# yanyan-li/PlanarSLAM

Measured on NVIDIA H100. Metric: rgbd_frames_per_sec_640x480, higher is better.
Workload: dtype u8/f64

## Files before the change

planarslam_b200/csrc/peac_kernels.cuh:

```cuda
#pragma once
#include <cuda_runtime.h>

#include <cfloat>
#include <cstdint>

#include "pslam_internal.h"

namespace pslam {

#define PEAC_MAX_PLANES 128
#define PEAC_PL_WORDS (PEAC_MAX_PLANES / 32)

__device__ __forceinline__ void eig33sym_jacobi(const double K[3][3], double s[3], double V[3][3]) {
    double a[3][3], d[3], b[3], z[3];
#pragma unroll
    for (int i = 0; i < 3; ++i) {
#pragma unroll
        for (int j = 0; j < 3; ++j) { a[i][j] = K[i][j]; V[i][j] = (i == j) ? 1.0 : 0.0; }
        d[i] = b[i] = a[i][i];
        z[i] = 0.0;
    }
    for (int sweep = 0; sweep < 50; ++sweep) {
        const double sm = fabs(a[0][1]) + fabs(a[0][2]) + fabs(a[1][2]);
        if (sm == 0.0) break;
        const double tresh = (sweep < 3) ? 0.2 * sm / 9.0 : 0.0;
#pragma unroll
        for (int p = 0; p < 2; ++p)
#pragma unroll
            for (int q = p + 1; q < 3; ++q) {
                const double g = 100.0 * fabs(a[p][q]);
                if (sweep > 3 && fabs(d[p]) + g == fabs(d[p]) && fabs(d[q]) + g == fabs(d[q])) {
                    a[p][q] = 0.0;
                } else if (fabs(a[p][q]) > tresh) {
                    double h = d[q] - d[p], t;
                    if (fabs(h) + g == fabs(h)) {
                        t = a[p][q] / h;
                    } else {
                        const double theta = 0.5 * h / a[p][q];
                        t = 1.0 / (fabs(theta) + sqrt(1.0 + theta * theta));
                        if (theta < 0.0) t = -t;
                    }
                    const double c = 1.0 / sqrt(1.0 + t * t), sn = t * c, tau = sn / (1.0 + c);
                    h = t * a[p][q];
                    z[p] -= h; z[q] += h; d[p] -= h; d[q] += h;
                    a[p][q] = 0.0;
#define PEAC_ROT(i, j, k, l) { const double gg = a[i][j], hh = a[k][l]; a[i][j] = gg - sn * (hh + gg * tau); a[k][l] = hh + sn * (gg - hh * tau); }
                    if (p == 0 && q == 1) { PEAC_ROT(0, 2, 1, 2) }
                    else if (p == 0 && q == 2) { PEAC_ROT(0, 1, 1, 2) }
                    else { PEAC_ROT(0, 1, 0, 2) }
#undef PEAC_ROT
#pragma unroll
                    for (int j = 0; j < 3; ++j) {
                        const double gg = V[j][p], hh = V[j][q];
                        V[j][p] = gg - sn * (hh + gg * tau);
                        V[j][q] = hh + sn * (gg - hh * tau);
                    }
                }
            }
#pragma unroll
        for (int i = 0; i < 3; ++i) { b[i] += z[i]; d[i] = b[i]; z[i] = 0.0; }
    }
#define PEAC_CSWAP(i, j) if (d[j] < d[i]) { double t_ = d[i]; d[i] = d[j]; d[j] = t_; \
        t_ = V[0][i]; V[0][i] = V[0][j]; V[0][j] = t_; t_ = V[1][i]; V[1][i] = V[1][j]; V[1][j] = t_; t_ = V[2][i]; V[2][i] = V[2][j]; V[2][j] = t_; }
    PEAC_CSWAP(0, 1)
    PEAC_CSWAP(0, 2)
    PEAC_CSWAP(1, 2)
#undef PEAC_CSWAP
    s[0] = d[0]; s[1] = d[1]; s[2] = d[2];
}

__device__ __forceinline__ void peac_stats_compute(const double st[9], int N, double geo[8]) {
    const double sc = 1.0 / N;
    const double sx = st[0], sy = st[1], sz = st[2];
    geo[0] = sx * sc; geo[1] = sy * sc; geo[2] = sz * sc;
    double K[3][3];
    K[0][0] = st[3] - sx * sx * sc; K[0][1] = st[6] - sx * sy * sc; K[0][2] = st[8] - sx * sz * sc;
    K[1][1] = st[4] - sy * sy * sc; K[1][2] = st[7] - sy * sz * sc; K[2][2] = st[5] - sz * sz * sc;
    K[1][0] = K[0][1]; K[2][0] = K[0][2]; K[2][1] = K[1][2];
    double sv[3], V[3][3];
    eig33sym_jacobi(K, sv, V);
    if (V[0][0] * geo[0] + V[1][0] * geo[1] + V[2][0] * geo[2] <= 0) { geo[3] = V[0][0]; geo[4] = V[1][0]; geo[5] = V[2][0]; }
    else { geo[3] = -V[0][0]; geo[4] = -V[1][0]; geo[5] = -V[2][0]; }
    geo[6] = sv[0] * sc;
    geo[7] = sv[0] / (sv[0] + sv[1] + sv[2]);
}

__device__ __forceinline__ double peac_t_mse(const PeacGeom& g, double tol, double z) { const double v = g.depth_sigma * z * z + tol; return v * v; }
__device__ __forceinline__ double peac_t_ang_init(const PeacGeom& g, double z) {
    if (z <= g.z_near) return g.t_ang_init_near;
    const double cz = fmin(z, g.z_far);
    const double factor = (g.angle_far - g.angle_near) / (g.z_far - g.z_near);
    return cos(factor * cz + g.angle_near - factor * g.z_near);
}
__device__ __forceinline__ double peac_sim(const double* ga, const double* gb) {
    return fabs(ga[3] * gb[3] + ga[4] * gb[4] + ga[5] * gb[5]);
}

__global__ void __launch_bounds__(128) k_peac_blocks(PeacGeom g, const uint16_t* __restrict__ depth, double* __restrict__ blk_st,
                                                     double* __restrict__ blk_geo, int32_t* __restrict__ blk_n, uint8_t* __restrict__ blk_valid) {
    const int b = blockIdx.x * 128 + threadIdx.x, frame = blockIdx.y;
    if (b >= g.nblk) return;
    const int bi = b / g.nbw, bj = b - bi * g.nbw;
    const uint16_t* D = depth + (size_t)frame * g.w * g.h;
    const double scale = (double)g.scale, fx = (double)g.fx, fy = (double)g.fy, cx = (double)g.cx, cy = (double)g.cy;
    double st[9] = {0, 0, 0, 0, 0, 0, 0, 0, 0};
    int n = 0;
    bool valid = true;
    for (int i = bi * g.win, ic = 0; ic < g.win && i < g.h && valid; ++i, ++ic)
        for (int j = bj * g.win, jc = 0; jc < g.win && j < g.w; ++j, ++jc) {
            const int dv = D[(size_t)i * g.w + j];
            if (dv == 0) { valid = false; break; }
            const double z = (double)dv * scale;
            const double tdz = g.depth_alpha * fabs(z) + g.depth_change_tol;
            if (j + 1 < g.w) { const int dn = D[(size_t)i * g.w + j + 1]; if (dn != 0 && fabs(z - (double)dn * scale) > tdz) { valid = false; break; } }
            if (i + 1 < g.h) { const int dn = D[(size_t)(i + 1) * g.w + j]; if (dn != 0 && fabs(z - (double)dn * scale) > tdz) { valid = false; break; } }
            const double x = ((double)j - cx) * z / fx, y = ((double)i - cy) * z / fy;
            st[0] += x; st[1] += y; st[2] += z;
            st[3] += x * x; st[4] += y * y; st[5] += z * z;
            st[6] += x * y; st[7] += y * z; st[8] += x * z;
            ++n;
        }
    double geo[8] = {0, 0, 0, 0, 0, 0, 0, 0};
    bool keep = false;
    if (!valid) { n = 0; for (int k = 0; k < 9; ++k) st[k] = 0; }
    if (n >= 4) {
        peac_stats_compute(st, n, geo);
        keep = valid && geo[6] < peac_t_mse(g, g.std_tol_init, geo[2]);
    } else {
        geo[6] = geo[7] = __longlong_as_double(0x7ff8000000000000LL);
    }
    const size_t o = (size_t)frame * g.nblk + b;
    for (int k = 0; k < 9; ++k) blk_st[o * 9 + k] = st[k];
    for (int k = 0; k < 8; ++k) blk_geo[o * 8 + k] = geo[k];
    blk_n[o] = n;
    blk_valid[o] = keep ? 1 : 0;
}

struct AhcState {
    int nslots;
    int words;
    double* st;
    double* geo;
    int32_t* N;
    int32_t* rid;
    int32_t* cid;
    uint8_t* alive;
    uint32_t* adj;
    int16_t* wlo;
    int16_t* whi;
    uint16_t* heap;
    float* keyf;
    int32_t* nb_list;
    int32_t* ds_parent;
    int32_t* ds_size;
};

__device__ __forceinline__ int ds_find(int32_t* parent, int x) {
    int r = x;
    while (parent[r] != r) r = parent[r];
    while (parent[x] != r) { const int nx = parent[x]; parent[x] = r; x = nx; }
    return r;
}
__device__ __forceinline__ void ds_union(int32_t* parent, int32_t* size, int x, int y) {
    const int xr = ds_find(parent, x), yr = ds_find(parent, y);
    if (xr == yr) return;
    if (size[xr] < size[yr]) { parent[xr] = yr; size[yr] += size[xr]; }
    else { parent[yr] = xr; size[xr] += size[yr]; }
}

struct HeapKey {
    const float* kf; const double* geo;
    __device__ __forceinline__ bool comp(int a, int b) const {
        const float fa = kf[a], fb = kf[b];
        if (fb < fa) return true;
        if (fb > fa) return false;
        return geo[(size_t)b * 8 + 6] < geo[(size_t)a * 8 + 6];
    }
};
__device__ __forceinline__ void heap_sift_up(uint16_t* h, const HeapKey& key, int hole, int top, int value) {
    int parent = (hole - 1) / 2;
    while (hole > top && key.comp(h[parent], value)) { h[hole] = h[parent]; hole = parent; parent = (hole - 1) / 2; }
    h[hole] = (uint16_t)value;
}
__device__ __forceinline__ void heap_push(uint16_t* h, int& len, const HeapKey& key, int id) { h[len] = (uint16_t)id; ++len; heap_sift_up(h, key, len - 1, 0, id); }
__device__ __forceinline__ int heap_pop(uint16_t* h, int& len, const HeapKey& key) {
    const int top = h[0], value = h[len - 1];
    --len;
    if (len > 0) {
        int hole = 0, child = 0;
        while (child < (len - 1) / 2) {
            child = 2 * (child + 1);
            if (key.comp(h[child], h[child - 1])) --child;
            h[hole] = h[child]; hole = child;
        }
        if ((len & 1) == 0 && child == (len - 2) / 2) { child = 2 * (child + 1); h[hole] = h[child - 1]; hole = child - 1; }
        heap_sift_up(h, key, hole, 0, value);
    }
    return top;
}

__device__ void ahc_run(const PeacGeom& g, AhcState S, int heap_len, int& next_cid, uint16_t* ex, const int exs, int& n_ex, bool& overflow) {
    const int lane = threadIdx.x & 31;
    const uint32_t full = 0xffffffffu;
    const HeapKey hkey{S.keyf, S.geo};
    int step = 0;
    while (heap_len > 0 && step <= g.max_step) {
        int p = 0;
        if (lane == 0) p = heap_pop(S.heap, heap_len, hkey);
        p = __shfl_sync(full, p, 0);
        heap_len = __shfl_sync(full, heap_len, 0);
        if (!S.alive[p]) continue;
        const int plo = S.wlo[p], phi = S.whi[p];
        int cnt = 0;
        for (int w0 = plo; w0 <= phi; w0 += 32) {
            const int w = w0 + lane;
            uint32_t bits = (w <= phi) ? S.adj[(size_t)p * S.words + w] : 0u;
            const int c = __popc(bits);
            int inc = c;
#pragma unroll
            for (int o = 1; o < 32; o <<= 1) { const int t = __shfl_up_sync(full, inc, o); if (lane >= o) inc += t; }
            int pos = cnt + inc - c;
            while (bits) { const int bpos = __ffs(bits) - 1; bits &= bits - 1; S.nb_list[pos++] = w * 32 + bpos; }
            cnt += __shfl_sync(full, inc, 31);
        }
        __syncwarp();
        const double* gp = S.geo + (size_t)p * 8;
        const double* sp = S.st + (size_t)p * 9;
        const int Np = S.N[p];
        double bst[9], bgeo[8];
        int best_nb = -1, best_cid = 0x7fffffff, best_N = 0;
#pragma unroll
        for (int k = 0; k < 8; ++k) bgeo[k] = 0;
        for (int i = lane; i < cnt; i += 32) {
            const int q = S.nb_list[i];
            const double* gq = S.geo + (size_t)q * 8;
            if (peac_sim(gp, gq) < g.sim_merge) continue;
            double st[9], geo[8];
            const double* sq = S.st + (size_t)q * 9;
#pragma unroll
            for (int k = 0; k < 9; ++k) st[k] = sp[k] + sq[k];
            const int Nq = S.N[q];
            peac_stats_compute(st, Np + Nq, geo);
            const int cq = S.cid[q];
            if (best_nb < 0 || geo[6] < bgeo[6] || (geo[6] == bgeo[6] && cq < best_cid)) {
                best_nb = q; best_cid = cq; best_N = Np + Nq;
#pragma unroll
                for (int k = 0; k < 9; ++k) bst[k] = st[k];
#pragma unroll
                for (int k = 0; k < 8; ++k) bgeo[k] = geo[k];
            }
        }
        double w_mse = bgeo[6];
        int w_nb = best_nb, w_cid = best_cid;
#pragma unroll
        for (int o = 16; o; o >>= 1) {
            const double om = __shfl_xor_sync(full, w_mse, o);
            const int onb = __shfl_xor_sync(full, w_nb, o), oc = __shfl_xor_sync(full, w_cid, o);
            if (onb >= 0 && (w_nb < 0 || om < w_mse || (om == w_mse && oc < w_cid))) { w_mse = om; w_nb = onb; w_cid = oc; }
        }
        bool merged = false;
        if (w_nb >= 0) {
            const int nb = w_nb;
            const int src = __ffs(__ballot_sync(full, best_nb == nb)) - 1;
            double st[9], geo[8];
#pragma unroll
            for (int k = 0; k < 9; ++k) st[k] = __shfl_sync(full, bst[k], src);
#pragma unroll
            for (int k = 0; k < 8; ++k) geo[k] = __shfl_sync(full, bgeo[k], src);
            const int Nc = __shfl_sync(full, best_N, src);
            if (geo[6] < peac_t_mse(g, g.std_tol_merge, geo[2])) {
                merged = true;
                const int rid_c = Np >= S.N[nb] ? S.rid[p] : S.rid[nb];
                if (lane == 0) ds_union(S.ds_parent, S.ds_size, S.rid[p], S.rid[nb]);
                const int nlo = S.wlo[nb], nhi = S.whi[nb];
                for (int w = nlo + lane; w <= nhi; w += 32) {
                    uint32_t bits = S.adj[(size_t)nb * S.words + w];
                    while (bits) {
                        const int q = w * 32 + __ffs(bits) - 1;
                        bits &= bits - 1;
                        if (q == p) continue;
                        atomicAnd(&S.adj[(size_t)q * S.words + (nb >> 5)], ~(1u << (nb & 31)));
                        atomicOr(&S.adj[(size_t)q * S.words + (p >> 5)], 1u << (p & 31));
                        if ((p >> 5) < S.wlo[q]) S.wlo[q] = (int16_t)(p >> 5);
                        if ((p >> 5) > S.whi[q]) S.whi[q] = (int16_t)(p >> 5);
                    }
                }
                __syncwarp();
                const int clo = min(plo, nlo), chi = max(phi, nhi);
                for (int w = clo + lane; w <= chi; w += 32) {
                    uint32_t u = S.adj[(size_t)p * S.words + w] | S.adj[(size_t)nb * S.words + w];
                    if (w == (p >> 5)) u &= ~(1u << (p & 31));
                    if (w == (nb >> 5)) u &= ~(1u << (nb & 31));
                    S.adj[(size_t)p * S.words + w] = u;
                    S.adj[(size_t)nb * S.words + w] = 0u;
                }
                if (lane == 0) {
#pragma unroll
                    for (int k = 0; k < 9; ++k) S.st[(size_t)p * 9 + k] = st[k];
#pragma unroll
                    for (int k = 0; k < 8; ++k) S.geo[(size_t)p * 8 + k] = geo[k];
                    S.N[p] = Nc; S.rid[p] = rid_c; S.cid[p] = next_cid; S.alive[nb] = 0; S.keyf[p] = (float)geo[6];
                    S.wlo[p] = (int16_t)clo; S.whi[p] = (int16_t)chi;
                }
                ++next_cid;
                __syncwarp();
                if (lane == 0) heap_push(S.heap, heap_len, hkey, p);
                heap_len = __shfl_sync(full, heap_len, 0);
            }
        }
        if (!merged) {
            if (Np >= g.min_support) { if (n_ex < PEAC_MAX_PLANES) { if (lane == 0) ex[n_ex * exs] = (uint16_t)p; ++n_ex; } else overflow = true; }
            for (int w = plo + lane; w <= phi; w += 32) {
                uint32_t bits = S.adj[(size_t)p * S.words + w];
                while (bits) { const int q = w * 32 + __ffs(bits) - 1; bits &= bits - 1; atomicAnd(&S.adj[(size_t)q * S.words + (p >> 5)], ~(1u << (p & 31))); }
                S.adj[(size_t)p * S.words + w] = 0u;
            }
            if (lane == 0) S.alive[p] = 0;
        }
        __syncwarp();
        ++step;
    }
    while (heap_len > 0) {
        int p = 0;
        if (lane == 0) p = heap_pop(S.heap, heap_len, hkey);
        p = __shfl_sync(full, p, 0);
        heap_len = __shfl_sync(full, heap_len, 0);
        if (S.alive[p] && S.N[p] >= g.min_support) { if (n_ex < PEAC_MAX_PLANES) { if (lane == 0) ex[n_ex * exs] = (uint16_t)p; ++n_ex; } else overflow = true; }
    }
    __syncwarp();
    if (lane == 0)
        for (int i = 1; i < n_ex; ++i) {
            const int v = ex[i * exs];
            int j = i - 1;
            while (j >= 0 && S.N[ex[j * exs]] < S.N[v]) { ex[(j + 1) * exs] = ex[j * exs]; --j; }
            ex[(j + 1) * exs] = (uint16_t)v;
        }
    __syncwarp();
}

struct PeacPlaneRec {
    double normal[3], center[3], mse, curvature;
    double st[9];
    int32_t N, rid, cid, valid;
};

template <int OCC>
__global__ void __launch_bounds__(32, OCC) k_peac_cluster(PeacGeom g, const double* __restrict__ blk_st, const double* __restrict__ blk_geo,
                                                     const int32_t* __restrict__ blk_n, const uint8_t* __restrict__ blk_valid,
                                                     double* node_st, double* node_geo, int32_t* node_n, int32_t* node_rid, int32_t* node_cid,
                                                     uint8_t* node_alive, uint32_t* adj, int16_t* wlo_all, int16_t* whi_all, int32_t* nb_list, int32_t* ds_parent,
                                                     int32_t* ds_size, PeacPlaneRec* planes, int32_t* n_planes, int32_t* blk_map,
                                                     int32_t* next_cid_out, int32_t* status, float* keyf_all) {
    const int frame = blockIdx.x, lane = threadIdx.x;
    const size_t fo = (size_t)frame * g.nblk;
    AhcState S;
    S.nslots = g.nblk; S.words = g.adj_words;
    S.st = node_st + fo * 9; S.geo = node_geo + fo * 8; S.N = node_n + fo; S.rid = node_rid + fo; S.cid = node_cid + fo;
    extern __shared__ __align__(16) unsigned char cluster_smem[];
    if (OCC > 12) {
        S.keyf = keyf_all + fo;
        S.heap = reinterpret_cast<uint16_t*>(cluster_smem);
    } else {
        S.keyf = reinterpret_cast<float*>(cluster_smem);
        S.heap = reinterpret_cast<uint16_t*>(cluster_smem + (size_t)g.nblk * sizeof(float));
    }
    S.alive = node_alive + fo; S.adj = adj + fo * g.adj_words; S.nb_list = nb_list + fo;
    S.wlo = wlo_all + fo; S.whi = whi_all + fo;
    S.ds_parent = ds_parent + fo; S.ds_size = ds_size + fo;
    const uint8_t* valid = blk_valid + fo;
    for (int b = lane; b < g.nblk; b += 32) {
        for (int k = 0; k < 9; ++k) S.st[(size_t)b * 9 + k] = blk_st[(fo + b) * 9 + k];
        for (int k = 0; k < 8; ++k) S.geo[(size_t)b * 8 + k] = blk_geo[(fo + b) * 8 + k];
        S.N[b] = blk_n[fo + b]; S.rid[b] = b; S.cid[b] = b; S.alive[b] = valid[b];
        S.ds_parent[b] = b; S.ds_size[b] = 1;
        S.keyf[b] = (float)blk_geo[(fo + b) * 8 + 6];
        S.wlo[b] = (int16_t)(max(b - g.nbw, 0) >> 5); S.whi[b] = (int16_t)(min(b + g.nbw, g.nblk - 1) >> 5);
    }
    __syncwarp();
    auto connect = [&](int a, int b) {
        atomicOr(&S.adj[(size_t)a * S.words + (b >> 5)], 1u << (b & 31));
        atomicOr(&S.adj[(size_t)b * S.words + (a >> 5)], 1u << (a & 31));
    };
    const int Nh = g.nbh, Nw = g.nbw;
    for (int i = lane; i < Nh; i += 32)
        for (int j = 1; j < Nw; j += 2) {
            const int c = i * Nw + j;
            if (!valid[c - 1]) { --j; continue; }
            if (!valid[c]) continue;
            if (j < Nw - 1 && !valid[c + 1]) { ++j; continue; }
            const double th = peac_t_ang_init(g, S.geo[(size_t)c * 8 + 2]);
            if ((j < Nw - 1 && peac_sim(S.geo + (size_t)(c - 1) * 8, S.geo + (size_t)(c + 1) * 8) >= th) ||
                (j == Nw - 1 && peac_sim(S.geo + (size_t)c * 8, S.geo + (size_t)(c - 1) * 8) >= th)) {
                connect(c, c - 1);
                if (j < Nw - 1) connect(c, c + 1);
            } else {
                --j;
            }
        }
    for (int j = lane; j < Nw; j += 32)
        for (int i = 1; i < Nh; i += 2) {
            const int c = i * Nw + j;
            if (!valid[c - Nw]) { --i; continue; }
            if (!valid[c]) continue;
            if (i < Nh - 1 && !valid[c + Nw]) { ++i; continue; }
            const double th = peac_t_ang_init(g, S.geo[(size_t)c * 8 + 2]);
            if ((i < Nh - 1 && peac_sim(S.geo + (size_t)(c - Nw) * 8, S.geo + (size_t)(c + Nw) * 8) >= th) ||
                (i == Nh - 1 && peac_sim(S.geo + (size_t)c * 8, S.geo + (size_t)(c - Nw) * 8) >= th)) {
                connect(c, c - Nw);
                if (i < Nh - 1) connect(c, c + Nw);
            } else {
                --i;
            }
        }
    __syncwarp();
    int heap_len = 0;
    if (lane == 0)
        { const HeapKey hkey{S.keyf, S.geo}; for (int b = 0; b < g.nblk; ++b) if (valid[b]) heap_push(S.heap, heap_len, hkey, b); }
    heap_len = __shfl_sync(0xffffffffu, heap_len, 0);
    __syncwarp();

    uint16_t* ex = S.heap + (g.nblk - 1);
    int n_ex = 0, next_cid = g.nblk;
    bool overflow = false;
    ahc_run(g, S, heap_len, next_cid, ex, -1, n_ex, overflow);
    if (overflow && lane == 0) atomicOr(status + frame, 16);

    PeacPlaneRec* P = planes + (size_t)frame * PEAC_MAX_PLANES;
    for (int i = lane; i < n_ex; i += 32) {
        const int s = ex[-i];
        PeacPlaneRec r;
        for (int k = 0; k < 3; ++k) { r.center[k] = S.geo[(size_t)s * 8 + k]; r.normal[k] = S.geo[(size_t)s * 8 + 3 + k]; }
        r.mse = S.geo[(size_t)s * 8 + 6]; r.curvature = S.geo[(size_t)s * 8 + 7];
        for (int k = 0; k < 9; ++k) r.st[k] = S.st[(size_t)s * 9 + k];
        r.N = S.N[s]; r.rid = S.rid[s]; r.cid = S.cid[s]; r.valid = 0;
        P[i] = r;
    }
    __syncwarp();
    int32_t* bm = blk_map + fo;
    const int PP = g.win * g.win;
    for (int b = lane; b < g.nblk; b += 32) {
        const int i = b / Nw, j = b - i * Nw;
        const int setid = ds_find(S.ds_parent, b);
        int plid = -1;
        if (S.ds_size[setid] * PP >= g.min_support) {
            bool same = true;
            if (j > 0 && ds_find(S.ds_parent, b - 1) != setid) same = false;
            if (same && j < Nw - 1 && ds_find(S.ds_parent, b + 1) != setid) same = false;
            if (same && i > 0 && ds_find(S.ds_parent, b - Nw) != setid) same = false;
            if (same && i < Nh - 1 && ds_find(S.ds_parent, b + Nw) != setid) same = false;
            if (same) {
                plid = 0;
                for (int k = 0; k < n_ex; ++k) if (P[k].rid == setid) { plid = k; break; }
                P[plid].valid = 1;
            }
        }
        bm[b] = plid;
    }
    if (lane == 0) { n_planes[frame] = n_ex; next_cid_out[frame] = next_cid; }
}

__device__ __forceinline__ int peac_seed_count(const PeacGeom& g, const int32_t* bm, int b) {
    const int i = b / g.nbw, j = b - i * g.nbw, W = g.win;
    int n = 0;
    if (bm[b] < 0) {
        if (i > 0 && bm[b - g.nbw] >= 0) n += W - 1;
        if (j > 0 && bm[b - 1] >= 0) n += W - 1;
    } else {
        if (i > 0 && bm[b - g.nbw] != bm[b]) n += W - 1;
        if (j > 0 && bm[b - 1] != bm[b]) n += W - 1;
    }
    return n;
}

__host__ __device__ __forceinline__ uint32_t peac_q_pack(int x, int y, uint32_t plane) { return (uint32_t)x | ((uint32_t)y << 12) | (plane << 24); }

__global__ void __launch_bounds__(256) k_peac_seed(PeacGeom g, const int32_t* __restrict__ blk_map, int32_t* __restrict__ labels,
                                                   float* __restrict__ dist, uint32_t* __restrict__ queue, int32_t* __restrict__ q_len) {
    const int frame = blockIdx.x, tid = threadIdx.x;
    const int32_t* bm = blk_map + (size_t)frame * g.nblk;
    int32_t* lab = labels + (size_t)frame * g.w * g.h;
    float* dm = dist + (size_t)frame * g.w * g.h;
    uint32_t* q = queue + (size_t)frame * g.queue_cap;
    const int npx = g.w * g.h;
    for (int p = tid; p < npx; p += 256) {
        const int y = p / g.w, x = p - y * g.w;
        const int by = y / g.win, bx = x / g.win;
        lab[p] = (by < g.nbh && bx < g.nbw) ? (bm[by * g.nbw + bx] >= 0 ? bm[by * g.nbw + bx] : -1) : -1;
        dm[p] = FLT_MAX;
    }
    __shared__ int s_part[256];
    const int per = (g.nblk + 255) / 256;
    const int b0 = tid * per, b1 = min(g.nblk, b0 + per);
    int mine = 0;
    for (int b = b0; b < b1; ++b) mine += peac_seed_count(g, bm, b);
    s_part[tid] = mine;
    __syncthreads();
    if (tid == 0) { int run = 0; for (int t = 0; t < 256; ++t) { const int v = s_part[t]; s_part[t] = run; run += v; } q_len[frame] = run; }
    __syncthreads();
    int pos = s_part[tid];
    const int W = g.win;
    for (int b = b0; b < b1; ++b) {
        const int i = b / g.nbw, j = b - i * g.nbw;
        if (bm[b] < 0) {
            if (i > 0 && bm[b - g.nbw] >= 0) { const uint32_t pl = (uint32_t)bm[b - g.nbw]; for (int k = 1; k < W; ++k) q[pos++] = peac_q_pack(j * W + k, i * W - 1, pl); }
            if (j > 0 && bm[b - 1] >= 0) { const uint32_t pl = (uint32_t)bm[b - 1]; for (int k = 0; k < W - 1; ++k) q[pos++] = peac_q_pack(j * W - 1, i * W + k, pl); }
        } else {
            const uint32_t pl = (uint32_t)bm[b];
            if (i > 0 && bm[b - g.nbw] != bm[b]) { for (int k = 0; k < W - 1; ++k) q[pos++] = peac_q_pack(j * W + k, i * W, pl); }
            if (j > 0 && bm[b - 1] != bm[b]) { for (int k = 1; k < W; ++k) q[pos++] = peac_q_pack(j * W, i * W + k, pl); }
        }
    }
}

struct FloodPlane { double n[3], c[3], th; };

__global__ void __launch_bounds__(32) k_peac_flood(PeacGeom g, const uint16_t* __restrict__ depth, const int32_t* __restrict__ blk_map,
                                                   const PeacPlaneRec* __restrict__ planes, const int32_t* __restrict__ n_planes,
                                                   int32_t* __restrict__ labels, float* __restrict__ dist,
                                                   uint32_t* __restrict__ queue, int32_t* __restrict__ q_len, uint32_t* __restrict__ pl_adj,
                                                   int32_t* __restrict__ status) {
    extern __shared__ __align__(16) unsigned char flood_smem[];
    FloodPlane* sP = reinterpret_cast<FloodPlane*>(flood_smem);
    int8_t* sbm = reinterpret_cast<int8_t*>(flood_smem + PEAC_MAX_PLANES * sizeof(FloodPlane));
    const int frame = blockIdx.x, lane = threadIdx.x;
    const uint32_t full = 0xffffffffu;
    const uint16_t* D = depth + (size_t)frame * g.w * g.h;
    const int32_t* bm = blk_map + (size_t)frame * g.nblk;
    const PeacPlaneRec* P = planes + (size_t)frame * PEAC_MAX_PLANES;
    int32_t* lab = labels + (size_t)frame * g.w * g.h;
    float* dm = dist + (size_t)frame * g.w * g.h;
    uint32_t* q = queue + (size_t)frame * g.queue_cap;
    uint32_t* padj = pl_adj + (size_t)frame * PEAC_MAX_PLANES * PEAC_PL_WORDS;
    const int np = n_planes[frame];
    for (int i = lane; i < np; i += 32) {
        FloodPlane f;
        for (int k = 0; k < 3; ++k) { f.n[k] = P[i].normal[k]; f.c[k] = P[i].center[k]; }
        f.th = 9 * P[i].mse + 1e-5;
        sP[i] = f;
    }
    for (int b = lane; b < g.nblk; b += 32) sbm[b] = (int8_t)bm[b];
    __syncwarp();
    int tail = q_len[frame];
    const double scale = (double)g.scale, fx = (double)g.fx, fy = (double)g.fy, cx = (double)g.cx, cy = (double)g.cy;
    const int item_in_group = lane >> 2, nbr = lane & 3;
    const uint32_t lt_mask = (1u << lane) - 1;
    bool overflow = false;

    struct Touch { int c, x, y, plid; float cdist; bool have, ok; };
    auto a_geom = [&](uint32_t e) -> Touch {
        Touch t;
        const int sx = e & 0xfff, sy = (e >> 12) & 0xfff;
        t.plid = e >> 24; t.c = -1; t.x = 0; t.y = 0; t.cdist = -1.f; t.ok = false; t.have = false;
        int n = nbr;
        if (sx > 0) { if (n == 0) { t.x = sx - 1; t.y = sy; t.have = true; } --n; }
        if (sx < g.w - 1) { if (n == 0 && !t.have) { t.x = sx + 1; t.y = sy; t.have = true; } --n; }
        if (sy > 0) { if (n == 0 && !t.have) { t.x = sx; t.y = sy - 1; t.have = true; } --n; }
        if (sy < g.h - 1) { if (n == 0 && !t.have) { t.x = sx; t.y = sy + 1; t.have = true; } --n; }
        if (t.have) {
            const int by = (t.y * g.win_magic) >> 16, bx = (t.x * g.win_magic) >> 16;
            if (by < g.nbh && bx < g.nbw && sbm[by * g.nbw + bx] >= 0) t.have = false;
        }
        if (t.have) t.c = t.y * g.w + t.x;
        return t;
    };
    auto a_math = [&](Touch& t, int dv) {
        if (t.have && dv != 0) {
            const FloodPlane& pr = sP[t.plid];
            const double z = (double)dv * scale;
            const double x = ((double)t.x - cx) * z / fx, y = ((double)t.y - cy) * z / fy;
            const double sd = pr.n[0] * (x - pr.c[0]) + pr.n[1] * (y - pr.c[1]) + pr.n[2] * (z - pr.c[2]);
            t.cdist = (float)fabs(sd);
            t.ok = (double)t.cdist * (double)t.cdist < pr.th;
        }
    };

    Touch nxt;
    nxt.c = -1; nxt.x = nxt.y = nxt.plid = 0; nxt.cdist = -1.f; nxt.have = nxt.ok = false;
    int nxt_dv = 0;
    uint32_t e_far = 0;
    bool next_ready = false, far_ready = false;
    for (int head = 0; head < tail;) {
        const int group = min(8, tail - head);
        const int k = head + item_in_group;
        Touch t = nxt;
        if (next_ready) a_math(t, nxt_dv);
        else {
            t.have = false; t.c = -1;
            if (item_in_group < group) { t = a_geom(q[k]); a_math(t, t.have ? (int)D[t.c] : 0); }
        }
        int tr = 0;
        float old = 0.f;
        if (t.have) { tr = lab[t.c]; old = dm[t.c]; }
        const bool whole_next = group == 8 && head + 16 <= tail;
        if (whole_next) {
            nxt = a_geom(far_ready ? e_far : q[k + 8]);
            nxt_dv = nxt.have ? (int)D[nxt.c] : 0;
            if (nxt.have) {
                asm volatile("prefetch.global.L1 [%0];" ::"l"(lab + nxt.c));
                asm volatile("prefetch.global.L1 [%0];" ::"l"(dm + nxt.c));
            }
        }
        next_ready = whole_next;
        far_ready = group == 8 && head + 24 <= tail;
        if (far_ready) e_far = q[k + 16];
        const uint32_t peers = __match_any_sync(full, t.have ? t.c : -1 - lane);
        const int rank = __popc(peers & lt_mask);
        int rounds = t.have ? __popc(peers) : 0;
#pragma unroll
        for (int o = 16; o; o >>= 1) rounds = max(rounds, __shfl_xor_sync(full, rounds, o));
        const int tr0 = tr;
        const float old0 = old;
        bool pushed = false;
        uint32_t rem = peers;
        for (int r = 0; r < rounds; ++r) {
            int ntr = tr;
            float nold = old;
            if (t.have && rank == r && tr > -6 && !(tr >= 0 && tr == t.plid)) {
                if (t.ok) {
                    if (tr >= 0) {
                        const FloodPlane& pr = sP[t.plid];
                        const FloodPlane& other = sP[tr];
                        const double sim = fabs(pr.n[0] * other.n[0] + pr.n[1] * other.n[1] + pr.n[2] * other.n[2]);
                        if (sim >= g.sim_refine) {
                            atomicOr(&padj[tr * PEAC_PL_WORDS + (t.plid >> 5)], 1u << (t.plid & 31));
                            atomicOr(&padj[t.plid * PEAC_PL_WORDS + (tr >> 5)], 1u << (tr & 31));
                        }
                    }
                    if (t.cdist < old) { ntr = t.plid; nold = t.cdist; pushed = true; }
                    else if (tr < 0) ntr = tr - 1;
                } else if (tr < 0) ntr = tr - 1;
            }
            const int src = rem ? (__ffs(rem) - 1) : lane;
            rem &= rem - 1;
            tr = __shfl_sync(full, ntr, src);
            old = __shfl_sync(full, nold, src);
        }
        if (t.have && rank == 0) {
            if (tr != tr0) lab[t.c] = tr;
            if (old != old0) dm[t.c] = old;
        }
        const uint32_t pm = __ballot_sync(full, pushed);
        if (pushed) {
            const int pos = tail + __popc(pm & lt_mask);
            if (pos < g.queue_cap) q[pos] = peac_q_pack(t.x, t.y, (uint32_t)t.plid); else overflow = true;
        }
        tail = min(tail + __popc(pm), g.queue_cap);
        head += group;
        __syncwarp();
    }
    if (__any_sync(full, overflow) && lane == 0) atomicOr(status + frame, 32);
    if (lane == 0) q_len[frame] = tail;
}

__global__ void __launch_bounds__(32) k_peac_final_merge(PeacGeom g, PeacPlaneRec* __restrict__ planes, const int32_t* __restrict__ n_planes,
                                                         const int32_t* __restrict__ next_cid_in, uint32_t* __restrict__ pl_adj,
                                                         int32_t* ds_parent, int32_t* ds_size, PeacPlaneRec* __restrict__ out_planes,
                                                         pslam_plane* __restrict__ abi_planes, int32_t* __restrict__ out_n,
                                                         int32_t* __restrict__ final_map, int32_t* __restrict__ status) {
    const int frame = blockIdx.x, tid = threadIdx.x;
    __shared__ double s_st[PEAC_MAX_PLANES * 9];
    __shared__ double s_geo[PEAC_MAX_PLANES * 8];
    __shared__ int32_t s_n[PEAC_MAX_PLANES], s_rid[PEAC_MAX_PLANES], s_cid[PEAC_MAX_PLANES], s_nb[PEAC_MAX_PLANES];
    __shared__ uint16_t s_heap[PEAC_MAX_PLANES];
    __shared__ uint8_t s_alive[PEAC_MAX_PLANES];
    __shared__ float s_key[PEAC_MAX_PLANES];
    __shared__ int16_t s_wlo[PEAC_MAX_PLANES], s_whi[PEAC_MAX_PLANES];
    __shared__ uint16_t s_ex[PEAC_MAX_PLANES];
    PeacPlaneRec* P = planes + (size_t)frame * PEAC_MAX_PLANES;
    PeacPlaneRec* O = out_planes + (size_t)frame * PEAC_MAX_PLANES;
    int32_t* fmap = final_map + (size_t)frame * PEAC_MAX_PLANES;
    const int np = n_planes[frame];
    const size_t fo = (size_t)frame * g.nblk;
    for (int i = tid; i < np; i += 32) {
        for (int k = 0; k < 9; ++k) s_st[i * 9 + k] = P[i].st[k];
        for (int k = 0; k < 3; ++k) { s_geo[i * 8 + k] = P[i].center[k]; s_geo[i * 8 + 3 + k] = P[i].normal[k]; }
        s_geo[i * 8 + 6] = P[i].mse; s_geo[i * 8 + 7] = P[i].curvature;
        s_n[i] = P[i].N; s_rid[i] = P[i].rid; s_cid[i] = P[i].cid; s_alive[i] = (uint8_t)P[i].valid;
        s_key[i] = (float)P[i].mse; s_wlo[i] = 0; s_whi[i] = PEAC_PL_WORDS - 1;
    }
    for (int i = tid; i < PEAC_MAX_PLANES; i += 32) fmap[i] = -1;
    __syncwarp();
    AhcState S;
    S.nslots = np; S.words = PEAC_PL_WORDS;
    S.st = s_st; S.geo = s_geo; S.N = s_n; S.rid = s_rid; S.cid = s_cid; S.alive = s_alive;
    S.adj = pl_adj + (size_t)frame * PEAC_MAX_PLANES * PEAC_PL_WORDS;
    S.heap = s_heap; S.keyf = s_key; S.wlo = s_wlo; S.whi = s_whi; S.nb_list = s_nb; S.ds_parent = ds_parent + fo; S.ds_size = ds_size + fo;
    int heap_len = 0;
    if (tid == 0) { const HeapKey hkey{S.keyf, S.geo}; for (int i = 0; i < np; ++i) if (s_alive[i]) heap_push(S.heap, heap_len, hkey, i); }
    heap_len = __shfl_sync(0xffffffffu, heap_len, 0);
    __syncwarp();
    int n_ex = 0, next_cid = next_cid_in[frame];
    bool overflow = false;
    ahc_run(g, S, heap_len, next_cid, s_ex, 1, n_ex, overflow);
    if (overflow && tid == 0) atomicOr(status + frame, 16);
    for (int j = tid; j < n_ex; j += 32) {
        const int s = s_ex[j];
        PeacPlaneRec r;
        for (int k = 0; k < 3; ++k) { r.center[k] = s_geo[s * 8 + k]; r.normal[k] = s_geo[s * 8 + 3 + k]; }
        r.mse = s_geo[s * 8 + 6]; r.curvature = s_geo[s * 8 + 7];
        for (int k = 0; k < 9; ++k) r.st[k] = s_st[s * 9 + k];
        r.N = s_n[s]; r.rid = s_rid[s]; r.cid = s_cid[s]; r.valid = 1;
        O[j] = r;
        pslam_plane a;
        for (int k = 0; k < 3; ++k) { a.normal[k] = r.normal[k]; a.center[k] = r.center[k]; }
        a.mse = r.mse; a.curvature = r.curvature; a.N = r.N; a.rid = r.rid;
        abi_planes[(size_t)frame * PEAC_MAX_PLANES + j] = a;
    }
    __syncwarp();
    if (tid == 0) {
        for (int i = 0; i < np; ++i) {
            if (!P[i].valid) continue;
            const int root = ds_find(S.ds_parent, P[i].rid);
            for (int j = 0; j < n_ex; ++j) if (O[j].rid == root) { fmap[i] = j; break; }
        }
        out_n[frame] = n_ex;
    }
}

#define PEAC_SUB 1024
#define PEAC_SUB_WARPS 4
__host__ __device__ inline int peac_num_sub(const PeacGeom& g) { return (g.w * g.h + PEAC_SUB - 1) / PEAC_SUB; }
__device__ __forceinline__ int peac_final_id(const int32_t* __restrict__ s_map, int v) { return (v >= 0 && v < PEAC_MAX_PLANES) ? s_map[v] : -1; }

__global__ void __launch_bounds__(32 * PEAC_SUB_WARPS) k_peac_member_count(PeacGeom g, const int32_t* __restrict__ labels, const int32_t* __restrict__ final_map,
                                                                           const int32_t* __restrict__ out_n, int32_t* __restrict__ counts, int nsub) {
    __shared__ int32_t s_map[PEAC_MAX_PLANES];
    __shared__ int32_t s_cnt[PEAC_SUB_WARPS][PEAC_MAX_PLANES];
    const int frame = blockIdx.y, warp = threadIdx.x >> 5, lane = threadIdx.x & 31;
    const int sub = blockIdx.x * PEAC_SUB_WARPS + warp;
    const int npx = g.w * g.h;
    for (int i = threadIdx.x; i < PEAC_MAX_PLANES; i += blockDim.x) s_map[i] = final_map[(size_t)frame * PEAC_MAX_PLANES + i];
    for (int i = lane; i < PEAC_MAX_PLANES; i += 32) s_cnt[warp][i] = 0;
    __syncthreads();
    if (sub >= nsub) return;
    const int nf = out_n[frame];
    const int32_t* lab = labels + (size_t)frame * npx;
    const int p0 = sub * PEAC_SUB, p1 = min(npx, p0 + PEAC_SUB);
    for (int base = p0; base < p1; base += 32) {
        const int p = base + lane;
        const int nv = (p < p1) ? peac_final_id(s_map, lab[p]) : -1;
        const uint32_t peers = __match_any_sync(0xffffffffu, nv);
        if (nv >= 0 && (peers & ((1u << lane) - 1)) == 0) s_cnt[warp][nv] += __popc(peers);
        __syncwarp();
    }
    int32_t* out = counts + ((size_t)frame * nsub + sub) * PEAC_MAX_PLANES;
    for (int k = lane; k < nf; k += 32) out[k] = s_cnt[warp][k];
}

__global__ void __launch_bounds__(PEAC_MAX_PLANES) k_peac_member_scan(const int32_t* __restrict__ out_n, int32_t* __restrict__ counts,
                                                                      int32_t* __restrict__ member_off, int nsub) {
    __shared__ int32_t s_tot[PEAC_MAX_PLANES];
    const int frame = blockIdx.x, k = threadIdx.x;
    const int nf = out_n[frame];
    int32_t* cf = counts + (size_t)frame * nsub * PEAC_MAX_PLANES;
    int run = 0;
    if (k < nf)
        for (int sb = 0; sb < nsub; ++sb) { const int v = cf[(size_t)sb * PEAC_MAX_PLANES + k]; cf[(size_t)sb * PEAC_MAX_PLANES + k] = run; run += v; }
    s_tot[k] = (k < nf) ? run : 0;
    __syncthreads();
    if (k == 0) {
        int32_t* moff = member_off + (size_t)frame * (PEAC_MAX_PLANES + 1);
        int acc = 0;
        for (int j = 0; j < nf; ++j) { moff[j] = acc; acc += s_tot[j]; }
        moff[nf] = acc;
    }
}

__global__ void __launch_bounds__(32 * PEAC_SUB_WARPS) k_peac_member_scatter(PeacGeom g, int32_t* __restrict__ labels, const int32_t* __restrict__ final_map,
                                                                             const int32_t* __restrict__ out_n, const int32_t* __restrict__ counts,
                                                                             const int32_t* __restrict__ member_off, int32_t* __restrict__ member_idx, int nsub) {
    __shared__ int32_t s_map[PEAC_MAX_PLANES];
    __shared__ int32_t s_pos[PEAC_SUB_WARPS][PEAC_MAX_PLANES];
    const int frame = blockIdx.y, warp = threadIdx.x >> 5, lane = threadIdx.x & 31;
    const int sub = blockIdx.x * PEAC_SUB_WARPS + warp;
    const int npx = g.w * g.h;
    for (int i = threadIdx.x; i < PEAC_MAX_PLANES; i += blockDim.x) s_map[i] = final_map[(size_t)frame * PEAC_MAX_PLANES + i];
    __syncthreads();
    if (sub >= nsub) return;
    const int nf = out_n[frame];
    const int32_t* base_cnt = counts + ((size_t)frame * nsub + sub) * PEAC_MAX_PLANES;
    const int32_t* moff = member_off + (size_t)frame * (PEAC_MAX_PLANES + 1);
    for (int k = lane; k < nf; k += 32) s_pos[warp][k] = moff[k] + base_cnt[k];
    __syncwarp();
    int32_t* lab = labels + (size_t)frame * npx;
    int32_t* midx = member_idx + (size_t)frame * npx;
    const int p0 = sub * PEAC_SUB, p1 = min(npx, p0 + PEAC_SUB);
    for (int base = p0; base < p1; base += 32) {
        const int p = base + lane;
        const int nv = (p < p1) ? peac_final_id(s_map, lab[p]) : -1;
        const uint32_t peers = __match_any_sync(0xffffffffu, nv);
        if (nv >= 0) {
            const int rank = __popc(peers & ((1u << lane) - 1));
            const int at = s_pos[warp][nv] + rank;
            lab[p] = nv;
            midx[at] = p;
        }
        __syncwarp();
        if (nv >= 0 && (peers & ((1u << lane) - 1)) == 0) s_pos[warp][nv] += __popc(peers);
        __syncwarp();
    }
}

}
```

planarslam_b200/csrc/peac_pipeline.cu:

```cuda
#include <algorithm>
#include <cmath>
#include <cstring>

#include "peac_kernels.cuh"

namespace pslam {

int peac_build_geometry(pslam_ctx* c) {
    const pslam_config& cf = c->cfg;
    PeacGeom& g = c->pgeom;
    std::memset(&g, 0, sizeof(g));
    g.w = cf.width; g.h = cf.height; g.win = 10;
    g.nbw = g.w / g.win; g.nbh = g.h / g.win; g.nblk = g.nbw * g.nbh;
    g.min_support = 3000; g.max_step = 100000;
    g.adj_words = (g.nblk + 31) / 32;
    g.queue_cap = 2 * g.w * g.h;
    g.scale = cf.depth_scale; g.fx = cf.fx; g.fy = cf.fy; g.cx = cf.cx; g.cy = cf.cy;
    g.depth_sigma = 1.6e-6; g.std_tol_init = 5; g.std_tol_merge = 8;
    g.z_near = 500; g.z_far = 4000;
    g.angle_near = 15.0 * M_PI / 180.0; g.angle_far = 90.0 * M_PI / 180.0;
    {
        const double factor = (g.angle_far - g.angle_near) / (g.z_far - g.z_near);
        g.t_ang_init_near = std::cos(factor * g.z_near + g.angle_near - factor * g.z_near);
    }
    g.sim_merge = std::cos(60.0 * M_PI / 180.0);
    g.sim_refine = std::cos(30.0 * M_PI / 180.0);
    g.depth_alpha = 0.04; g.depth_change_tol = 0.02;
    if (g.w > 4096 || g.h > 4096) return set_error(c, PSLAM_E_INVALID, "frame larger than 4096 in one dimension (12-bit queue coordinates)");
    g.win_magic = (65536 + g.win - 1) / g.win;
    for (int x = 0; x < std::max(g.w, g.h); ++x)
        if (((x * g.win_magic) >> 16) != x / g.win) return set_error(c, PSLAM_E_INVALID, "block index reciprocal is not exact for this frame size");
    if (g.nblk < 1) return set_error(c, PSLAM_E_INVALID, "frame smaller than one PEAC block");
    if (g.nblk > 65535) return set_error(c, PSLAM_E_INVALID, "more than 65535 PEAC blocks per frame (the clustering heap holds 16-bit slot ids)");
    if (!(cf.fx != 0.f) || !(cf.fy != 0.f) || !(cf.depth_scale > 0.f)) return set_error(c, PSLAM_E_INVALID, "fx, fy must be non-zero and depth_scale > 0");
    return PSLAM_OK;
}

template <typename T>
static int dmalloc(pslam_ctx* c, T** p, size_t n) { return check_cuda(c, cudaMalloc((void**)p, std::max<size_t>(n, 1) * sizeof(T)), "cudaMalloc"); }

int peac_alloc(pslam_ctx* c) {
    const PeacGeom& g = c->pgeom;
    const size_t B = c->cfg.max_batch, nb = g.nblk, px = (size_t)g.w * g.h;
    int rc;
#define A(call) if ((rc = (call)) != PSLAM_OK) return rc
    A(dmalloc(c, &c->d_depth, B * px));
    A(dmalloc(c, &c->d_blk_st, B * nb * 9)); A(dmalloc(c, &c->d_blk_geo, B * nb * 8)); A(dmalloc(c, &c->d_blk_n, B * nb)); A(dmalloc(c, &c->d_blk_valid, B * nb));
    A(dmalloc(c, &c->d_node_st, B * nb * 9)); A(dmalloc(c, &c->d_node_geo, B * nb * 8)); A(dmalloc(c, &c->d_node_n, B * nb));
    A(dmalloc(c, &c->d_node_rid, B * nb)); A(dmalloc(c, &c->d_node_cid, B * nb)); A(dmalloc(c, &c->d_node_alive, B * nb));
    A(dmalloc(c, &c->d_adj, B * nb * g.adj_words)); A(dmalloc(c, &c->d_wlo, B * nb)); A(dmalloc(c, &c->d_whi, B * nb)); A(dmalloc(c, &c->d_nb_list, B * nb)); A(dmalloc(c, &c->d_keyf, B * nb));
    A(dmalloc(c, &c->d_ds_parent, B * nb)); A(dmalloc(c, &c->d_ds_size, B * nb));
    A(dmalloc(c, &c->d_coarse, B * PEAC_MAX_PLANES)); A(dmalloc(c, &c->d_ncoarse, B)); A(dmalloc(c, &c->d_next_cid, B)); A(dmalloc(c, &c->d_blk_map, B * nb));
    A(dmalloc(c, &c->d_dist, B * px)); A(dmalloc(c, &c->d_queue, B * g.queue_cap)); A(dmalloc(c, &c->d_qlen, B));
    A(dmalloc(c, &c->d_pl_adj, B * PEAC_MAX_PLANES * PEAC_PL_WORDS));
    A(dmalloc(c, &c->d_final, B * PEAC_MAX_PLANES)); A(dmalloc(c, &c->d_scratch, B * (size_t)peac_num_sub(g) * PEAC_MAX_PLANES));
    A(dmalloc(c, &c->d_final_map, B * PEAC_MAX_PLANES));
    A(dmalloc(c, &c->d_labels, B * px)); A(dmalloc(c, &c->d_planes, B * PEAC_MAX_PLANES)); A(dmalloc(c, &c->d_nplanes, B));
    A(dmalloc(c, &c->d_midx, B * px)); A(dmalloc(c, &c->d_moff, B * (PEAC_MAX_PLANES + 1)));
    A(check_cuda(c, cudaMallocHost((void**)&c->h_depth, B * px * sizeof(uint16_t)), "cudaMallocHost"));
#undef A
    c->peac_ready = true;
    return PSLAM_OK;
}

void peac_free(pslam_ctx* c) {
    cudaFree(c->d_depth); cudaFree(c->d_blk_st); cudaFree(c->d_blk_geo); cudaFree(c->d_blk_n); cudaFree(c->d_blk_valid);
    cudaFree(c->d_node_st); cudaFree(c->d_node_geo); cudaFree(c->d_node_n); cudaFree(c->d_node_rid); cudaFree(c->d_node_cid);
    cudaFree(c->d_node_alive); cudaFree(c->d_adj); cudaFree(c->d_wlo); cudaFree(c->d_whi); cudaFree(c->d_nb_list); cudaFree(c->d_keyf); cudaFree(c->d_ds_parent); cudaFree(c->d_ds_size);
    cudaFree(c->d_coarse); cudaFree(c->d_ncoarse); cudaFree(c->d_next_cid); cudaFree(c->d_blk_map); cudaFree(c->d_dist); cudaFree(c->d_queue);
    cudaFree(c->d_qlen); cudaFree(c->d_pl_adj); cudaFree(c->d_final); cudaFree(c->d_scratch); cudaFree(c->d_final_map); cudaFree(c->d_labels); cudaFree(c->d_planes);
    cudaFree(c->d_nplanes); cudaFree(c->d_midx); cudaFree(c->d_moff); cudaFreeHost(c->h_depth);
}

static int peac_cluster_occ() {
    static const int occ = [] { const char* e = std::getenv("PSLAM_PEAC_OCC"); const int v = e ? std::atoi(e) : 12; return (v == 16 || v == 20) ? v : 12; }();
    return occ;
}
static size_t peac_cluster_smem(const PeacGeom& g, int occ) {
    return (size_t)g.nblk * (occ > 12 ? sizeof(uint16_t) : sizeof(float) + sizeof(uint16_t));
}

int peac_run_dev(pslam_ctx* c, const uint16_t* d_depth, int nframes, int32_t* d_labels, pslam_plane* d_planes, int32_t* d_nplanes,
                 int32_t* d_member_idx, int32_t* d_member_off) {
    const PeacGeom& g = c->pgeom;
    if (nframes < 1 || nframes > c->cfg.max_batch) return set_error(c, PSLAM_E_INVALID, "nframes outside [1, max_batch]");
    if (!d_depth || !d_labels || !d_planes || !d_nplanes || !d_member_idx || !d_member_off) return set_error(c, PSLAM_E_INVALID, "null device pointer");
    if (!c->peac_ready) { const int arc = peac_alloc(c); if (arc != PSLAM_OK) return arc; }
    cudaStream_t st = c->stream;
    c->last_nframes = nframes;
    PSLAM_CUDA(c, cudaMemsetAsync(c->d_status, 0, nframes * sizeof(int32_t), st));
    PSLAM_CUDA(c, cudaMemsetAsync(c->d_adj, 0, (size_t)nframes * g.nblk * g.adj_words * sizeof(uint32_t), st));
    PSLAM_CUDA(c, cudaMemsetAsync(c->d_pl_adj, 0, (size_t)nframes * PEAC_MAX_PLANES * PEAC_PL_WORDS * sizeof(uint32_t), st));
    PSLAM_LAUNCH(c, "peac_blocks", k_peac_blocks<<<dim3((g.nblk + 127) / 128, nframes), 128, 0, st>>>(g, d_depth, c->d_blk_st, c->d_blk_geo, c->d_blk_n, c->d_blk_valid));
    const int occ = peac_cluster_occ();
    const size_t cluster_smem = peac_cluster_smem(g, occ);
#define PEAC_CLUSTER(V) do { \
        PSLAM_CUDA(c, cudaFuncSetAttribute(k_peac_cluster<V>, cudaFuncAttributeMaxDynamicSharedMemorySize, (int)cluster_smem)); \
        PSLAM_CUDA(c, cudaFuncSetAttribute(k_peac_cluster<V>, cudaFuncAttributePreferredSharedMemoryCarveout, cudaSharedmemCarveoutMaxShared)); \
        PSLAM_LAUNCH(c, "peac_cluster", k_peac_cluster<V><<<nframes, 32, cluster_smem, st>>>(g, c->d_blk_st, c->d_blk_geo, c->d_blk_n, c->d_blk_valid, c->d_node_st, \
                     c->d_node_geo, c->d_node_n, c->d_node_rid, c->d_node_cid, c->d_node_alive, c->d_adj, c->d_wlo, c->d_whi, c->d_nb_list, c->d_ds_parent, c->d_ds_size, \
                     c->d_coarse, c->d_ncoarse, c->d_blk_map, c->d_next_cid, c->d_status, c->d_keyf)); } while (0)
    if (occ == 16) PEAC_CLUSTER(16); else if (occ == 20) PEAC_CLUSTER(20); else PEAC_CLUSTER(12);
#undef PEAC_CLUSTER
    PSLAM_LAUNCH(c, "peac_seed", k_peac_seed<<<nframes, 256, 0, st>>>(g, c->d_blk_map, d_labels, c->d_dist, c->d_queue, c->d_qlen));
    const size_t flood_smem = PEAC_MAX_PLANES * sizeof(FloodPlane) + (size_t)g.nblk;
    PSLAM_CUDA(c, cudaFuncSetAttribute(k_peac_flood, cudaFuncAttributeMaxDynamicSharedMemorySize, (int)flood_smem));
    PSLAM_LAUNCH(c, "peac_flood", k_peac_flood<<<nframes, 32, flood_smem, st>>>(g, d_depth, c->d_blk_map, c->d_coarse, c->d_ncoarse, d_labels, c->d_dist, c->d_queue,
                 c->d_qlen, c->d_pl_adj, c->d_status));
    PSLAM_LAUNCH(c, "peac_final_merge", k_peac_final_merge<<<nframes, 32, 0, st>>>(g, c->d_coarse, c->d_ncoarse, c->d_next_cid, c->d_pl_adj, c->d_ds_parent,
                 c->d_ds_size, c->d_final, d_planes, d_nplanes, c->d_final_map, c->d_status));
    const int nsub = peac_num_sub(g);
    const dim3 mgrid((nsub + PEAC_SUB_WARPS - 1) / PEAC_SUB_WARPS, nframes);
    PSLAM_LAUNCH(c, "peac_member_count", k_peac_member_count<<<mgrid, 32 * PEAC_SUB_WARPS, 0, st>>>(g, d_labels, c->d_final_map, d_nplanes, c->d_scratch, nsub));
    PSLAM_LAUNCH(c, "peac_member_scan", k_peac_member_scan<<<nframes, PEAC_MAX_PLANES, 0, st>>>(d_nplanes, c->d_scratch, d_member_off, nsub));
    PSLAM_LAUNCH(c, "peac_member_scatter", k_peac_member_scatter<<<mgrid, 32 * PEAC_SUB_WARPS, 0, st>>>(g, d_labels, c->d_final_map, d_nplanes, c->d_scratch,
                 d_member_off, d_member_idx, nsub));
    PSLAM_CUDA(c, cudaGetLastError());
    return PSLAM_OK;
}

}

using namespace pslam;

extern "C" {

int pslam_peac_max_planes(const pslam_ctx*) { return PEAC_MAX_PLANES; }
int pslam_peac_num_blocks(const pslam_ctx* c) { return c ? c->pgeom.nblk : 0; }

int pslam_peac_wave_frames(const pslam_ctx* c) {
    if (!c) return 0;
    const int occ = peac_cluster_occ();
    const size_t cluster_smem = peac_cluster_smem(c->pgeom, occ);
    int per_sm = 0, sms = 0, dev = 0;
    if (cudaGetDevice(&dev) != cudaSuccess) return 0;
#define PEAC_OCCUPANCY(V) do { \
        if (cudaFuncSetAttribute(k_peac_cluster<V>, cudaFuncAttributeMaxDynamicSharedMemorySize, (int)cluster_smem) != cudaSuccess) return 0; \
        cudaFuncSetAttribute(k_peac_cluster<V>, cudaFuncAttributePreferredSharedMemoryCarveout, cudaSharedmemCarveoutMaxShared); \
        if (cudaOccupancyMaxActiveBlocksPerMultiprocessor(&per_sm, k_peac_cluster<V>, 32, cluster_smem) != cudaSuccess) return 0; } while (0)
    if (occ == 16) PEAC_OCCUPANCY(16); else if (occ == 20) PEAC_OCCUPANCY(20); else PEAC_OCCUPANCY(12);
#undef PEAC_OCCUPANCY
    if (cudaDeviceGetAttribute(&sms, cudaDevAttrMultiProcessorCount, dev) != cudaSuccess) return 0;
    return per_sm * sms;
}

int pslam_peac_run_batch_dev(pslam_ctx* c, const uint16_t* d_depth, int nframes, int32_t* d_labels, pslam_plane* d_planes, int32_t* d_nplanes,
                             int32_t* d_member_idx, int32_t* d_member_off) {
    if (!c) return PSLAM_E_INVALID;
    PSLAM_CUDA(c, cudaSetDevice(c->cfg.device));
    return peac_run_dev(c, d_depth, nframes, d_labels, d_planes, d_nplanes, d_member_idx, d_member_off);
}

int pslam_peac_run_batch(pslam_ctx* c, const uint16_t* depth, int nframes, int32_t* labels, pslam_plane* planes, int32_t* nplanes,
                         int32_t* member_idx, int32_t* member_off) {
    if (!c) return PSLAM_E_INVALID;
    if (!depth || !labels || !planes || !nplanes) return set_error(c, PSLAM_E_INVALID, "null pointer");
    if (nframes < 1 || nframes > c->cfg.max_batch) return set_error(c, PSLAM_E_INVALID, "nframes outside [1, max_batch]");
    PSLAM_CUDA(c, cudaSetDevice(c->cfg.device));
    if (!c->peac_ready) { const int arc = peac_alloc(c); if (arc != PSLAM_OK) return arc; }
    const PeacGeom& g = c->pgeom;
    const size_t px = (size_t)g.w * g.h;
    cudaStream_t st = c->stream;
    const uint16_t* src = depth;
    if (!host_ptr_is_pinned(depth)) { std::memcpy(c->h_depth, depth, px * nframes * sizeof(uint16_t)); src = c->h_depth; }
    PSLAM_CUDA(c, cudaMemcpyAsync(c->d_depth, src, px * nframes * sizeof(uint16_t), cudaMemcpyHostToDevice, st));
    int rc = peac_run_dev(c, c->d_depth, nframes, c->d_labels, c->d_planes, c->d_nplanes, c->d_midx, c->d_moff);
    if (rc != PSLAM_OK) return rc;
    PSLAM_CUDA(c, cudaMemcpyAsync(labels, c->d_labels, px * nframes * sizeof(int32_t), cudaMemcpyDeviceToHost, st));
    PSLAM_CUDA(c, cudaMemcpyAsync(planes, c->d_planes, (size_t)nframes * PEAC_MAX_PLANES * sizeof(pslam_plane), cudaMemcpyDeviceToHost, st));
    PSLAM_CUDA(c, cudaMemcpyAsync(nplanes, c->d_nplanes, nframes * sizeof(int32_t), cudaMemcpyDeviceToHost, st));
    if (member_idx) PSLAM_CUDA(c, cudaMemcpyAsync(member_idx, c->d_midx, px * nframes * sizeof(int32_t), cudaMemcpyDeviceToHost, st));
    if (member_off) PSLAM_CUDA(c, cudaMemcpyAsync(member_off, c->d_moff, (size_t)nframes * (PEAC_MAX_PLANES + 1) * sizeof(int32_t), cudaMemcpyDeviceToHost, st));
    PSLAM_CUDA(c, cudaMemcpyAsync(c->h_status, c->d_status, nframes * sizeof(int32_t), cudaMemcpyDeviceToHost, st));
    PSLAM_CUDA(c, cudaStreamSynchronize(st));
    int bits = 0;
    for (int i = 0; i < nframes; ++i) bits |= c->h_status[i];
    if (bits) return set_error(c, PSLAM_E_CAPACITY, "PEAC capacity exceeded (16: more than PEAC_MAX_PLANES planes, 32: region-growing queue)");
    return PSLAM_OK;
}

int pslam_peac_debug_blocks(pslam_ctx* c, int frame, double* st9, double* geo8, int32_t* n, uint8_t* valid) {
    if (!c || !c->peac_ready || frame < 0 || frame >= c->last_nframes) return PSLAM_E_INVALID;
    PSLAM_CUDA(c, cudaStreamSynchronize(c->stream));
    const size_t nb = c->pgeom.nblk, o = (size_t)frame * nb;
    if (st9) PSLAM_CUDA(c, cudaMemcpy(st9, c->d_blk_st + o * 9, nb * 9 * sizeof(double), cudaMemcpyDeviceToHost));
    if (geo8) PSLAM_CUDA(c, cudaMemcpy(geo8, c->d_blk_geo + o * 8, nb * 8 * sizeof(double), cudaMemcpyDeviceToHost));
    if (n) PSLAM_CUDA(c, cudaMemcpy(n, c->d_blk_n + o, nb * sizeof(int32_t), cudaMemcpyDeviceToHost));
    if (valid) PSLAM_CUDA(c, cudaMemcpy(valid, c->d_blk_valid + o, nb, cudaMemcpyDeviceToHost));
    return PSLAM_OK;
}

int pslam_peac_debug_coarse(pslam_ctx* c, int frame, int32_t* blk_map, int32_t* n_coarse) {
    if (!c || !c->peac_ready || frame < 0 || frame >= c->last_nframes) return PSLAM_E_INVALID;
    PSLAM_CUDA(c, cudaStreamSynchronize(c->stream));
    const size_t nb = c->pgeom.nblk;
    if (blk_map) PSLAM_CUDA(c, cudaMemcpy(blk_map, c->d_blk_map + (size_t)frame * nb, nb * sizeof(int32_t), cudaMemcpyDeviceToHost));
    if (n_coarse) PSLAM_CUDA(c, cudaMemcpy(n_coarse, c->d_ncoarse + frame, sizeof(int32_t), cudaMemcpyDeviceToHost));
    return PSLAM_OK;
}

}
```

planarslam_b200/csrc/pslam_internal.h:

```cpp
#pragma once
#include <cuda.h>
#include <cuda_runtime.h>

#include <cstdint>
#include <string>
#include <vector>

#include "../../include/pslam_abi.h"

#define PSLAM_MAX_LEVELS 8

namespace pslam {

struct LevelGeom {
    int w, h, pitch;
    int pyr_off;
    int blur_off, blur_pitch;
    int n_cols, n_rows;
    int w_cell, h_cell;
    int max_bx, max_by;
    int cell_base;
    int slot_cap;
    int slot_base;
    int quota;
    int kp_cap;
    int kp_base;
    int cand_cap;
    int cand_base;
    int node_cap, node_base;
    int tabx_off, taby_off;
    int n_ini; float h_x;
    int work_base;
    float scale;
    int patch_size;
};

struct OrbGeom {
    int nlevels;
    int width, height;
    int total_cells, total_slots, total_kp, total_cand, total_nodes, total_work, total_tabx, total_taby;
    int pyr_bytes;
    LevelGeom lv[PSLAM_MAX_LEVELS];
    int ini_th, min_th;
    int umax[16];
};

#define BT_W 128
#define BT_H 64
#define BT_BOX_W 160
#define BT_X_PAD 16
#define BT_BOX_H 70
struct BlurTmaParams {
    CUtensorMap map[PSLAM_MAX_LEVELS];
    int tile_base[PSLAM_MAX_LEVELS + 1];
    int tiles_x[PSLAM_MAX_LEVELS];
    int w[PSLAM_MAX_LEVELS], h[PSLAM_MAX_LEVELS], dst_pitch[PSLAM_MAX_LEVELS], dst_off[PSLAM_MAX_LEVELS];
    int nlevels;
};

struct PeacGeom {
    int w, h, nbw, nbh, nblk, win;
    int win_magic;
    int min_support, max_step;
    int adj_words, queue_cap;
    float scale, fx, fy, cx, cy;
    double depth_sigma, std_tol_init, std_tol_merge;
    double z_near, z_far, angle_near, angle_far, t_ang_init_near;
    double sim_merge, sim_refine;
    double depth_alpha, depth_change_tol;
};

struct PeacPlaneRec;
struct PoseBuffers;
struct SearchBuffers;
struct LbaBuffers;
struct LsdBuffers;
struct TrackBuffers;
struct ExchangeBuffers;
struct PlanePostBuffers;
struct BowDbBuffers;
struct FrameBuffers;

}

struct pslam_ctx {
    pslam_config cfg;
    pslam::OrbGeom geom;
    std::vector<float> scale, inv_scale, sigma2, inv_sigma2;
    std::vector<int> quota;
    cudaStream_t own_stream = nullptr, stream = nullptr;
    int64_t launches = 0;
    bool profile = false;
    struct ProfRec { const char* name; cudaEvent_t a, b; };
    std::vector<ProfRec> prof;
    std::string err;
    int last_nframes = 0;
    bool orb_ready = false, peac_ready = false;

    uint8_t* d_gray = nullptr;
    const uint8_t* d_gray_cur = nullptr;
    uint8_t* d_pyr = nullptr;
    uint8_t* d_blur = nullptr;
    int blur_frame_bytes = 0;
    pslam::BlurTmaParams blur_tma;
    const uint8_t* blur_tma_src = nullptr; int blur_tma_n = 0;
    CUtensorMap* d_blur_maps = nullptr;
    int16_t* d_xofs = nullptr; int16_t* d_xa = nullptr;
    int16_t* d_yofs = nullptr; int16_t* d_ya = nullptr;
    uint32_t* d_slots = nullptr;
    int32_t* d_cell_cnt = nullptr;
    uint32_t* d_cand = nullptr;
    int32_t* d_cand_cnt = nullptr;
    int4* d_nodes = nullptr;
    int2* d_links = nullptr;
    int32_t* d_work = nullptr;
    uint32_t* d_lvl_kp = nullptr;
    int32_t* d_lvl_cnt = nullptr;
    int32_t* d_status = nullptr;
    pslam_keypoint* d_kps = nullptr;
    uint8_t* d_desc = nullptr;
    int32_t* d_n = nullptr;
    pslam::PeacGeom pgeom;
    uint16_t* d_depth = nullptr;
    double* d_blk_st = nullptr; double* d_blk_geo = nullptr; int32_t* d_blk_n = nullptr; uint8_t* d_blk_valid = nullptr;
    double* d_node_st = nullptr; double* d_node_geo = nullptr; int32_t* d_node_n = nullptr; int32_t* d_node_rid = nullptr;
    int32_t* d_node_cid = nullptr; uint8_t* d_node_alive = nullptr; uint32_t* d_adj = nullptr; int16_t* d_wlo = nullptr; int16_t* d_whi = nullptr;
    int32_t* d_nb_list = nullptr; float* d_keyf = nullptr; int32_t* d_ds_parent = nullptr; int32_t* d_ds_size = nullptr;
    pslam::PeacPlaneRec* d_coarse = nullptr; int32_t* d_ncoarse = nullptr; int32_t* d_next_cid = nullptr; int32_t* d_blk_map = nullptr;
    float* d_dist = nullptr; uint32_t* d_queue = nullptr; int32_t* d_qlen = nullptr; uint32_t* d_pl_adj = nullptr;
    pslam::PeacPlaneRec* d_final = nullptr; int32_t* d_scratch = nullptr; int32_t* d_final_map = nullptr;
    int32_t* d_labels = nullptr; pslam_plane* d_planes = nullptr; int32_t* d_nplanes = nullptr; int32_t* d_midx = nullptr; int32_t* d_moff = nullptr;
    uint16_t* h_depth = nullptr;
    pslam::PoseBuffers* pose = nullptr;
    pslam::SearchBuffers* search = nullptr;
    pslam::LbaBuffers* lba = nullptr;
    pslam::LsdBuffers* lsd = nullptr;
    pslam::TrackBuffers* track = nullptr;
    pslam::PlanePostBuffers* planepost = nullptr;
    pslam::FrameBuffers* frame = nullptr;
    pslam::BowDbBuffers* bowdb = nullptr;
    pslam::ExchangeBuffers* exchange = nullptr;
    uint8_t* h_gray = nullptr; pslam_keypoint* h_kps = nullptr; uint8_t* h_desc = nullptr; int32_t* h_n = nullptr;
    int32_t* h_status = nullptr;
};

namespace pslam {
int set_error(pslam_ctx* c, int code, const std::string& msg);
int check_cuda(pslam_ctx* c, cudaError_t e, const char* what);
int orb_build_geometry(pslam_ctx* c);
int orb_alloc(pslam_ctx* c);
void orb_free(pslam_ctx* c);
int orb_run_dev(pslam_ctx* c, const uint8_t* d_gray, int nframes, pslam_keypoint* d_kps, uint8_t* d_desc, int cap,
                int32_t* d_n);
void pose_free(pslam_ctx* c);
void search_free(pslam_ctx* c);
void lba_free(pslam_ctx* c);
void lsd_free(pslam_ctx* c);
void track_free(pslam_ctx* c);
void exchange_free(pslam_ctx* c);
void planepost_free(pslam_ctx* c);
void bowdb_free(pslam_ctx* c);
void frame_free(pslam_ctx* c);
int lsd_status_fetch_async(pslam_ctx* c, int nframes, int32_t* h_pinned);
int peac_build_geometry(pslam_ctx* c);
int peac_alloc(pslam_ctx* c);
void peac_free(pslam_ctx* c);
int peac_run_dev(pslam_ctx* c, const uint16_t* d_depth, int nframes, int32_t* d_labels, pslam_plane* d_planes, int32_t* d_nplanes,
                 int32_t* d_member_idx, int32_t* d_member_off);
}

#define PSLAM_LAUNCH(c, name, ...)                                            \
    do {                                                                      \
        pslam_ctx::ProfRec _r{name, nullptr, nullptr};                        \
        if ((c)->profile) { cudaEventCreate(&_r.a); cudaEventCreate(&_r.b); cudaEventRecord(_r.a, (c)->stream); } \
        __VA_ARGS__;                                                          \
        if ((c)->profile) { cudaEventRecord(_r.b, (c)->stream); (c)->prof.push_back(_r); } \
        ++(c)->launches;                                                      \
    } while (0)

static inline bool host_ptr_is_pinned(const void* p) {
    cudaPointerAttributes a;
    if (cudaPointerGetAttributes(&a, p) != cudaSuccess) { cudaGetLastError(); return false; }
    return a.type == cudaMemoryTypeHost;
}

#define PSLAM_CUDA(c, call)                                                   \
    do {                                                                      \
        int _rc = pslam::check_cuda((c), (call), #call);                      \
        if (_rc != PSLAM_OK) return _rc;                                      \
    } while (0)
```

Before: 5173.

## Pack PEAC cluster node state into 128-byte AoS records and fuse merge loops

Replaces the separate struct-of-arrays node buffers (st, geo, N, rid, cid, alive, wlo, whi) used by agglomerative clustering with one 128-byte aligned hot record per node plus a cold record holding center and curvature. The neighbour-list materialisation step is replaced by warp-shuffle k-th-set-bit lookup, the two adjacency update loops in a merge are fused into one, and heap keys are stored alongside heap ids. The aim is fewer scattered cache lines per node access and fewer passes and warp syncs in the serial merge loop. In exchange, nodes take more memory, wlo/whi updates become atomics, and the occupancy template choice is removed.

```diff
diff --git a/planarslam_b200/csrc/peac_kernels.cuh b/planarslam_b200/csrc/peac_kernels.cuh
--- a/planarslam_b200/csrc/peac_kernels.cuh
+++ b/planarslam_b200/csrc/peac_kernels.cuh
@@ -92,9 +92,10 @@
     const double factor = (g.angle_far - g.angle_near) / (g.z_far - g.z_near);
     return cos(factor * cz + g.angle_near - factor * g.z_near);
 }
-__device__ __forceinline__ double peac_sim(const double* ga, const double* gb) {
-    return fabs(ga[3] * gb[3] + ga[4] * gb[4] + ga[5] * gb[5]);
-}
+__device__ __forceinline__ double peac_sim_n(const double* na, const double* nb) {
+    return fabs(na[0] * nb[0] + na[1] * nb[1] + na[2] * nb[2]);
+}
+__device__ __forceinline__ double peac_sim(const double* ga, const double* gb) { return peac_sim_n(ga + 3, gb + 3); }
 
 __global__ void __launch_bounds__(128) k_peac_blocks(PeacGeom g, const uint16_t* __restrict__ depth, double* __restrict__ blk_st,
                                                      double* __restrict__ blk_geo, int32_t* __restrict__ blk_n, uint8_t* __restrict__ blk_valid) {
@@ -136,24 +137,37 @@
     blk_valid[o] = keep ? 1 : 0;
 }
 
+struct __align__(128) PeacNode {
+    double st[9];
+    double normal[3];
+    double mse;
+    int32_t N, cid, rid;
+    int32_t wlo, whi;
+    int32_t alive;
+};
+static_assert(sizeof(PeacNode) == 128, "one node per 128-byte line");
+struct PeacNodeCold { double center[3], curvature; };
+
 struct AhcState {
     int nslots;
     int words;
-    double* st;
-    double* geo;
-    int32_t* N;
-    int32_t* rid;
-    int32_t* cid;
-    uint8_t* alive;
+    PeacNode* node;
+    PeacNodeCold* cold;
     uint32_t* adj;
-    int16_t* wlo;
-    int16_t* whi;
     uint16_t* heap;
-    float* keyf;
-    int32_t* nb_list;
+    float* heap_key;
     int32_t* ds_parent;
     int32_t* ds_size;
 };
+
+__device__ __forceinline__ void peac_node_set(PeacNode& n, PeacNodeCold& c, const double st[9], const double geo[8], int N, int cid, int rid) {
+#pragma unroll
+    for (int k = 0; k < 9; ++k) n.st[k] = st[k];
+#pragma unroll
+    for (int k = 0; k < 3; ++k) { n.normal[k] = geo[3 + k]; c.center[k] = geo[k]; }
+    n.mse = geo[6]; c.curvature = geo[7];
+    n.N = N; n.cid = cid; n.rid = rid;
+}
 
 __device__ __forceinline__ int ds_find(int32_t* parent, int x) {
     int r = x;
@@ -167,87 +181,110 @@
     if (size[xr] < size[yr]) { parent[xr] = yr; size[yr] += size[xr]; }
     else { parent[yr] = xr; size[xr] += size[yr]; }
 }
-
-struct HeapKey {
-    const float* kf; const double* geo;
-    __device__ __forceinline__ bool comp(int a, int b) const {
-        const float fa = kf[a], fb = kf[b];
+__device__ __forceinline__ void ds_union_loaded(int32_t* parent, int32_t* size, int x, int y, int px, int py, int sx, int sy) {
+    if (px != x || py != y) { ds_union(parent, size, x, y); return; }
+    if (x == y) return;
+    if (sx < sy) { parent[x] = y; size[y] = sy + sx; }
+    else { parent[y] = x; size[x] = sx + sy; }
+}
+
+struct AhcHeap {
+    uint16_t* id;
+    float* key;
+    const PeacNode* node;
+    __device__ __forceinline__ bool comp(int a, float fa, int b, float fb) const {
         if (fb < fa) return true;
         if (fb > fa) return false;
-        return geo[(size_t)b * 8 + 6] < geo[(size_t)a * 8 + 6];
+        return node[b].mse < node[a].mse;
+    }
+    __device__ __forceinline__ void sift_up(int hole, int top, int value, float vkey) const {
+        int parent = (hole - 1) / 2;
+        while (hole > top && comp(id[parent], key[parent], value, vkey)) { id[hole] = id[parent]; key[hole] = key[parent]; hole = parent; parent = (hole - 1) / 2; }
+        id[hole] = (uint16_t)value; key[hole] = vkey;
+    }
+    __device__ __forceinline__ void push(int& len, int value, float vkey) const { ++len; sift_up(len - 1, 0, value, vkey); }
+    __device__ __forceinline__ int pop(int& len) const {
+        const int top = id[0], value = id[len - 1];
+        const float vkey = key[len - 1];
+        --len;
+        if (len > 0) {
+            int hole = 0, child = 0;
+            while (child < (len - 1) / 2) {
+                child = 2 * (child + 1);
+                if (comp(id[child], key[child], id[child - 1], key[child - 1])) --child;
+                id[hole] = id[child]; key[hole] = key[child]; hole = child;
+            }
+            if ((len & 1) == 0 && child == (len - 2) / 2) { child = 2 * (child + 1); id[hole] = id[child - 1]; key[hole] = key[child - 1]; hole = child - 1; }
+            sift_up(hole, 0, value, vkey);
+        }
+        return top;
+    }
+    template <typename F>
+    __device__ __forceinline__ int build(int n, F take) const {
+        int len = 0;
+        for (int i = 0; i < n; ++i) if (take(i)) push(len, i, key[i]);
+        return len;
     }
 };
-__device__ __forceinline__ void heap_sift_up(uint16_t* h, const HeapKey& key, int hole, int top, int value) {
-    int parent = (hole - 1) / 2;
-    while (hole > top && key.comp(h[parent], value)) { h[hole] = h[parent]; hole = parent; parent = (hole - 1) / 2; }
-    h[hole] = (uint16_t)value;
-}
-__device__ __forceinline__ void heap_push(uint16_t* h, int& len, const HeapKey& key, int id) { h[len] = (uint16_t)id; ++len; heap_sift_up(h, key, len - 1, 0, id); }
-__device__ __forceinline__ int heap_pop(uint16_t* h, int& len, const HeapKey& key) {
-    const int top = h[0], value = h[len - 1];
-    --len;
-    if (len > 0) {
-        int hole = 0, child = 0;
-        while (child < (len - 1) / 2) {
-            child = 2 * (child + 1);
-            if (key.comp(h[child], h[child - 1])) --child;
-            h[hole] = h[child]; hole = child;
-        }
-        if ((len & 1) == 0 && child == (len - 2) / 2) { child = 2 * (child + 1); h[hole] = h[child - 1]; hole = child - 1; }
-        heap_sift_up(h, key, hole, 0, value);
-    }
-    return top;
-}
-
+
+__device__ __forceinline__ int peac_kth_slot(uint32_t bits, int inc, int w0, int k, int total) {
+    int j = 0;
+#pragma unroll
+    for (int s = 16; s; s >>= 1) { const int v = __shfl_sync(0xffffffffu, inc, j + s - 1); if (v <= k) j += s; }
+    uint32_t b = __shfl_sync(0xffffffffu, bits, j);
+    const int before = __shfl_sync(0xffffffffu, inc, (j + 31) & 31);
+    if (k >= total) return -1;
+    for (int r = k - (j ? before : 0); r > 0; --r) b &= b - 1;
+    return (w0 + j) * 32 + __ffs(b) - 1;
+}
+
+template <bool kGlobal>
 __device__ void ahc_run(const PeacGeom& g, AhcState S, int heap_len, int& next_cid, uint16_t* ex, const int exs, int& n_ex, bool& overflow) {
     const int lane = threadIdx.x & 31;
     const uint32_t full = 0xffffffffu;
-    const HeapKey hkey{S.keyf, S.geo};
+    const AhcHeap H{S.heap, S.heap_key, S.node};
     int step = 0;
     while (heap_len > 0 && step <= g.max_step) {
         int p = 0;
-        if (lane == 0) p = heap_pop(S.heap, heap_len, hkey);
+        if (lane == 0) {
+            p = H.pop(heap_len);
+            if (kGlobal && heap_len > 0) asm volatile("prefetch.global.L1 [%0];" ::"l"(S.node + S.heap[0]));
+        }
         p = __shfl_sync(full, p, 0);
         heap_len = __shfl_sync(full, heap_len, 0);
-        if (!S.alive[p]) continue;
-        const int plo = S.wlo[p], phi = S.whi[p];
-        int cnt = 0;
+        const PeacNode& np = S.node[p];
+        if (!np.alive) continue;
+        const int plo = np.wlo, phi = np.whi, Np = np.N, rid_p = np.rid;
+        const double* sp = np.st;
+        double bst[9], bgeo[8];
+        int best_nb = -1, best_cid = 0x7fffffff, best_N = 0, best_rid = 0, best_whi = 0, best_wlo = 0;
+#pragma unroll
+        for (int k = 0; k < 8; ++k) bgeo[k] = 0;
         for (int w0 = plo; w0 <= phi; w0 += 32) {
             const int w = w0 + lane;
-            uint32_t bits = (w <= phi) ? S.adj[(size_t)p * S.words + w] : 0u;
-            const int c = __popc(bits);
-            int inc = c;
+            const uint32_t bits = (w <= phi) ? S.adj[(size_t)p * S.words + w] : 0u;
+            int inc = __popc(bits);
 #pragma unroll
             for (int o = 1; o < 32; o <<= 1) { const int t = __shfl_up_sync(full, inc, o); if (lane >= o) inc += t; }
-            int pos = cnt + inc - c;
-            while (bits) { const int bpos = __ffs(bits) - 1; bits &= bits - 1; S.nb_list[pos++] = w * 32 + bpos; }
-            cnt += __shfl_sync(full, inc, 31);
-        }
-        __syncwarp();
-        const double* gp = S.geo + (size_t)p * 8;
-        const double* sp = S.st + (size_t)p * 9;
-        const int Np = S.N[p];
-        double bst[9], bgeo[8];
-        int best_nb = -1, best_cid = 0x7fffffff, best_N = 0;
-#pragma unroll
-        for (int k = 0; k < 8; ++k) bgeo[k] = 0;
-        for (int i = lane; i < cnt; i += 32) {
-            const int q = S.nb_list[i];
-            const double* gq = S.geo + (size_t)q * 8;
-            if (peac_sim(gp, gq) < g.sim_merge) continue;
-            double st[9], geo[8];
-            const double* sq = S.st + (size_t)q * 9;
-#pragma unroll
-            for (int k = 0; k < 9; ++k) st[k] = sp[k] + sq[k];
-            const int Nq = S.N[q];
-            peac_stats_compute(st, Np + Nq, geo);
-            const int cq = S.cid[q];
-            if (best_nb < 0 || geo[6] < bgeo[6] || (geo[6] == bgeo[6] && cq < best_cid)) {
-                best_nb = q; best_cid = cq; best_N = Np + Nq;
-#pragma unroll
-                for (int k = 0; k < 9; ++k) bst[k] = st[k];
-#pragma unroll
-                for (int k = 0; k < 8; ++k) bgeo[k] = geo[k];
+            const int total = __shfl_sync(full, inc, 31);
+            for (int k0 = 0; k0 < total; k0 += 32) {
+                const int q = peac_kth_slot(bits, inc, w0, k0 + lane, total);
+                if (q < 0) continue;
+                const PeacNode& nq = S.node[q];
+                if (peac_sim_n(np.normal, nq.normal) < g.sim_merge) continue;
+                double st[9], geo[8];
+#pragma unroll
+                for (int k = 0; k < 9; ++k) st[k] = sp[k] + nq.st[k];
+                const int Nq = nq.N;
+                peac_stats_compute(st, Np + Nq, geo);
+                const int cq = nq.cid;
+                if (best_nb < 0 || geo[6] < bgeo[6] || (geo[6] == bgeo[6] && cq < best_cid)) {
+                    best_nb = q; best_cid = cq; best_N = Np + Nq; best_rid = nq.rid; best_wlo = nq.wlo; best_whi = nq.whi;
+#pragma unroll
+                    for (int k = 0; k < 9; ++k) bst[k] = st[k];
+#pragma unroll
+                    for (int k = 0; k < 8; ++k) bgeo[k] = geo[k];
+                }
             }
         }
         double w_mse = bgeo[6];
@@ -268,43 +305,39 @@
 #pragma unroll
             for (int k = 0; k < 8; ++k) geo[k] = __shfl_sync(full, bgeo[k], src);
             const int Nc = __shfl_sync(full, best_N, src);
+            const int rid_nb = __shfl_sync(full, best_rid, src);
+            const int nlo = __shfl_sync(full, best_wlo, src), nhi = __shfl_sync(full, best_whi, src);
             if (geo[6] < peac_t_mse(g, g.std_tol_merge, geo[2])) {
                 merged = true;
-                const int rid_c = Np >= S.N[nb] ? S.rid[p] : S.rid[nb];
-                if (lane == 0) ds_union(S.ds_parent, S.ds_size, S.rid[p], S.rid[nb]);
-                const int nlo = S.wlo[nb], nhi = S.whi[nb];
-                for (int w = nlo + lane; w <= nhi; w += 32) {
+                const int rid_c = Np >= Nc - Np ? rid_p : rid_nb;
+                const int clo = min(plo, nlo), chi = max(phi, nhi);
+                int ds_px = 0, ds_py = 0, ds_sx = 0, ds_sy = 0;
+                if (lane == 0) { ds_px = S.ds_parent[rid_p]; ds_py = S.ds_parent[rid_nb]; ds_sx = S.ds_size[rid_p]; ds_sy = S.ds_size[rid_nb]; }
+                for (int w = clo + lane; w <= chi; w += 32) {
+                    const uint32_t up = S.adj[(size_t)p * S.words + w];
                     uint32_t bits = S.adj[(size_t)nb * S.words + w];
+                    uint32_t u = up | bits;
+                    if (w == (p >> 5)) { u &= ~(1u << (p & 31)); bits &= ~(1u << (p & 31)); }
+                    if (w == (nb >> 5)) u &= ~(1u << (nb & 31));
+                    S.adj[(size_t)p * S.words + w] = u;
+                    S.adj[(size_t)nb * S.words + w] = 0u;
                     while (bits) {
                         const int q = w * 32 + __ffs(bits) - 1;
                         bits &= bits - 1;
-                        if (q == p) continue;
                         atomicAnd(&S.adj[(size_t)q * S.words + (nb >> 5)], ~(1u << (nb & 31)));
                         atomicOr(&S.adj[(size_t)q * S.words + (p >> 5)], 1u << (p & 31));
-                        if ((p >> 5) < S.wlo[q]) S.wlo[q] = (int16_t)(p >> 5);
-                        if ((p >> 5) > S.whi[q]) S.whi[q] = (int16_t)(p >> 5);
+                        atomicMin(&S.node[q].wlo, p >> 5);
+                        atomicMax(&S.node[q].whi, p >> 5);
                     }
                 }
-                __syncwarp();
-                const int clo = min(plo, nlo), chi = max(phi, nhi);
-                for (int w = clo + lane; w <= chi; w += 32) {
-                    uint32_t u = S.adj[(size_t)p * S.words + w] | S.adj[(size_t)nb * S.words + w];
-                    if (w == (p >> 5)) u &= ~(1u << (p & 31));
-                    if (w == (nb >> 5)) u &= ~(1u << (nb & 31));
-                    S.adj[(size_t)p * S.words + w] = u;
-                    S.adj[(size_t)nb * S.words + w] = 0u;
-                }
                 if (lane == 0) {
-#pragma unroll
-                    for (int k = 0; k < 9; ++k) S.st[(size_t)p * 9 + k] = st[k];
-#pragma unroll
-                    for (int k = 0; k < 8; ++k) S.geo[(size_t)p * 8 + k] = geo[k];
-                    S.N[p] = Nc; S.rid[p] = rid_c; S.cid[p] = next_cid; S.alive[nb] = 0; S.keyf[p] = (float)geo[6];
-                    S.wlo[p] = (int16_t)clo; S.whi[p] = (int16_t)chi;
+                    peac_node_set(S.node[p], S.cold[p], st, geo, Nc, next_cid, rid_c);
+                    S.node[p].wlo = clo; S.node[p].whi = chi; S.node[nb].alive = 0;
+                    ds_union_loaded(S.ds_parent, S.ds_size, rid_p, rid_nb, ds_px, ds_py, ds_sx, ds_sy);
                 }
                 ++next_cid;
                 __syncwarp();
-                if (lane == 0) heap_push(S.heap, heap_len, hkey, p);
+                if (lane == 0) H.push(heap_len, p, (float)geo[6]);
                 heap_len = __shfl_sync(full, heap_len, 0);
             }
         }
@@ -315,24 +348,24 @@
                 while (bits) { const int q = w * 32 + __ffs(bits) - 1; bits &= bits - 1; atomicAnd(&S.adj[(size_t)q * S.words + (p >> 5)], ~(1u << (p & 31))); }
                 S.adj[(size_t)p * S.words + w] = 0u;
             }
-            if (lane == 0) S.alive[p] = 0;
+            if (lane == 0) S.node[p].alive = 0;
         }
         __syncwarp();
         ++step;
     }
     while (heap_len > 0) {
         int p = 0;
-        if (lane == 0) p = heap_pop(S.heap, heap_len, hkey);
+        if (lane == 0) p = H.pop(heap_len);
         p = __shfl_sync(full, p, 0);
         heap_len = __shfl_sync(full, heap_len, 0);
-        if (S.alive[p] && S.N[p] >= g.min_support) { if (n_ex < PEAC_MAX_PLANES) { if (lane == 0) ex[n_ex * exs] = (uint16_t)p; ++n_ex; } else overflow = true; }
+        if (S.node[p].alive && S.node[p].N >= g.min_support) { if (n_ex < PEAC_MAX_PLANES) { if (lane == 0) ex[n_ex * exs] = (uint16_t)p; ++n_ex; } else overflow = true; }
     }
     __syncwarp();
     if (lane == 0)
         for (int i = 1; i < n_ex; ++i) {
             const int v = ex[i * exs];
             int j = i - 1;
-            while (j >= 0 && S.N[ex[j * exs]] < S.N[v]) { ex[(j + 1) * exs] = ex[j * exs]; --j; }
+            while (j >= 0 && S.node[ex[j * exs]].N < S.node[v].N) { ex[(j + 1) * exs] = ex[j * exs]; --j; }
             ex[(j + 1) * exs] = (uint16_t)v;
         }
     __syncwarp();
@@ -344,37 +377,33 @@
     int32_t N, rid, cid, valid;
 };
 
-template <int OCC>
-__global__ void __launch_bounds__(32, OCC) k_peac_cluster(PeacGeom g, const double* __restrict__ blk_st, const double* __restrict__ blk_geo,
-                                                     const int32_t* __restrict__ blk_n, const uint8_t* __restrict__ blk_valid,
-                                                     double* node_st, double* node_geo, int32_t* node_n, int32_t* node_rid, int32_t* node_cid,
-                                                     uint8_t* node_alive, uint32_t* adj, int16_t* wlo_all, int16_t* whi_all, int32_t* nb_list, int32_t* ds_parent,
-                                                     int32_t* ds_size, PeacPlaneRec* planes, int32_t* n_planes, int32_t* blk_map,
-                                                     int32_t* next_cid_out, int32_t* status, float* keyf_all) {
+__global__ void __launch_bounds__(32, 12) k_peac_cluster(PeacGeom g, const double* __restrict__ blk_st, const double* __restrict__ blk_geo,
+                                                         const int32_t* __restrict__ blk_n, const uint8_t* __restrict__ blk_valid,
+                                                         PeacNode* node, PeacNodeCold* cold, uint32_t* adj, int32_t* ds_parent,
+                                                         int32_t* ds_size, PeacPlaneRec* planes, int32_t* n_planes, int32_t* blk_map,
+                                                         int32_t* next_cid_out, int32_t* status) {
     const int frame = blockIdx.x, lane = threadIdx.x;
     const size_t fo = (size_t)frame * g.nblk;
     AhcState S;
     S.nslots = g.nblk; S.words = g.adj_words;
-    S.st = node_st + fo * 9; S.geo = node_geo + fo * 8; S.N = node_n + fo; S.rid = node_rid + fo; S.cid = node_cid + fo;
+    S.node = node + fo; S.cold = cold + fo;
     extern __shared__ __align__(16) unsigned char cluster_smem[];
-    if (OCC > 12) {
-        S.keyf = keyf_all + fo;
-        S.heap = reinterpret_cast<uint16_t*>(cluster_smem);
-    } else {
-        S.keyf = reinterpret_cast<float*>(cluster_smem);
-        S.heap = reinterpret_cast<uint16_t*>(cluster_smem + (size_t)g.nblk * sizeof(float));
-    }
-    S.alive = node_alive + fo; S.adj = adj + fo * g.adj_words; S.nb_list = nb_list + fo;
-    S.wlo = wlo_all + fo; S.whi = whi_all + fo;
+    S.heap_key = reinterpret_cast<float*>(cluster_smem);
+    S.heap = reinterpret_cast<uint16_t*>(cluster_smem + (size_t)g.nblk * sizeof(float));
+    S.adj = adj + fo * g.adj_words;
     S.ds_parent = ds_parent + fo; S.ds_size = ds_size + fo;
     const uint8_t* valid = blk_valid + fo;
+    const double* bgeo = blk_geo + fo * 8;
     for (int b = lane; b < g.nblk; b += 32) {
-        for (int k = 0; k < 9; ++k) S.st[(size_t)b * 9 + k] = blk_st[(fo + b) * 9 + k];
-        for (int k = 0; k < 8; ++k) S.geo[(size_t)b * 8 + k] = blk_geo[(fo + b) * 8 + k];
-        S.N[b] = blk_n[fo + b]; S.rid[b] = b; S.cid[b] = b; S.alive[b] = valid[b];
+        double st[9], geo[8];
+        for (int k = 0; k < 9; ++k) st[k] = blk_st[(fo + b) * 9 + k];
+        for (int k = 0; k < 8; ++k) geo[k] = bgeo[(size_t)b * 8 + k];
+        PeacNode& n = S.node[b];
+        peac_node_set(n, S.cold[b], st, geo, blk_n[fo + b], b, b);
+        n.alive = valid[b];
+        n.wlo = max(b - g.nbw, 0) >> 5; n.whi = min(b + g.nbw, g.nblk - 1) >> 5;
         S.ds_parent[b] = b; S.ds_size[b] = 1;
-        S.keyf[b] = (float)blk_geo[(fo + b) * 8 + 6];
-        S.wlo[b] = (int16_t)(max(b - g.nbw, 0) >> 5); S.whi[b] = (int16_t)(min(b + g.nbw, g.nblk - 1) >> 5);
+        S.heap_key[b] = (float)geo[6];
     }
     __syncwarp();
     auto connect = [&](int a, int b) {
@@ -388,9 +417,9 @@
             if (!valid[c - 1]) { --j; continue; }
             if (!valid[c]) continue;
             if (j < Nw - 1 && !valid[c + 1]) { ++j; continue; }
-            const double th = peac_t_ang_init(g, S.geo[(size_t)c * 8 + 2]);
-            if ((j < Nw - 1 && peac_sim(S.geo + (size_t)(c - 1) * 8, S.geo + (size_t)(c + 1) * 8) >= th) ||
-                (j == Nw - 1 && peac_sim(S.geo + (size_t)c * 8, S.geo + (size_t)(c - 1) * 8) >= th)) {
+            const double th = peac_t_ang_init(g, bgeo[(size_t)c * 8 + 2]);
+            if ((j < Nw - 1 && peac_sim(bgeo + (size_t)(c - 1) * 8, bgeo + (size_t)(c + 1) * 8) >= th) ||
+                (j == Nw - 1 && peac_sim(bgeo + (size_t)c * 8, bgeo + (size_t)(c - 1) * 8) >= th)) {
                 connect(c, c - 1);
                 if (j < Nw - 1) connect(c, c + 1);
             } else {
@@ -403,9 +432,9 @@
             if (!valid[c - Nw]) { --i; continue; }
             if (!valid[c]) continue;
             if (i < Nh - 1 && !valid[c + Nw]) { ++i; continue; }
-            const double th = peac_t_ang_init(g, S.geo[(size_t)c * 8 + 2]);
-            if ((i < Nh - 1 && peac_sim(S.geo + (size_t)(c - Nw) * 8, S.geo + (size_t)(c + Nw) * 8) >= th) ||
-                (i == Nh - 1 && peac_sim(S.geo + (size_t)c * 8, S.geo + (size_t)(c - Nw) * 8) >= th)) {
+            const double th = peac_t_ang_init(g, bgeo[(size_t)c * 8 + 2]);
+            if ((i < Nh - 1 && peac_sim(bgeo + (size_t)(c - Nw) * 8, bgeo + (size_t)(c + Nw) * 8) >= th) ||
+                (i == Nh - 1 && peac_sim(bgeo + (size_t)c * 8, bgeo + (size_t)(c - Nw) * 8) >= th)) {
                 connect(c, c - Nw);
                 if (i < Nh - 1) connect(c, c + Nw);
             } else {
@@ -414,25 +443,26 @@
         }
     __syncwarp();
     int heap_len = 0;
-    if (lane == 0)
-        { const HeapKey hkey{S.keyf, S.geo}; for (int b = 0; b < g.nblk; ++b) if (valid[b]) heap_push(S.heap, heap_len, hkey, b); }
+    if (lane == 0) heap_len = AhcHeap{S.heap, S.heap_key, S.node}.build(g.nblk, [&](int b) { return valid[b] != 0; });
     heap_len = __shfl_sync(0xffffffffu, heap_len, 0);
     __syncwarp();
 
     uint16_t* ex = S.heap + (g.nblk - 1);
     int n_ex = 0, next_cid = g.nblk;
     bool overflow = false;
-    ahc_run(g, S, heap_len, next_cid, ex, -1, n_ex, overflow);
+    ahc_run<true>(g, S, heap_len, next_cid, ex, -1, n_ex, overflow);
     if (overflow && lane == 0) atomicOr(status + frame, 16);
 
     PeacPlaneRec* P = planes + (size_t)frame * PEAC_MAX_PLANES;
     for (int i = lane; i < n_ex; i += 32) {
         const int s = ex[-i];
         PeacPlaneRec r;
-        for (int k = 0; k < 3; ++k) { r.center[k] = S.geo[(size_t)s * 8 + k]; r.normal[k] = S.geo[(size_t)s * 8 + 3 + k]; }
-        r.mse = S.geo[(size_t)s * 8 + 6]; r.curvature = S.geo[(size_t)s * 8 + 7];
-        for (int k = 0; k < 9; ++k) r.st[k] = S.st[(size_t)s * 9 + k];
-        r.N = S.N[s]; r.rid = S.rid[s]; r.cid = S.cid[s]; r.valid = 0;
+        const PeacNode& n = S.node[s];
+        const PeacNodeCold& c = S.cold[s];
+        for (int k = 0; k < 3; ++k) { r.center[k] = c.center[k]; r.normal[k] = n.normal[k]; }
+        r.mse = n.mse; r.curvature = c.curvature;
+        for (int k = 0; k < 9; ++k) r.st[k] = n.st[k];
+        r.N = n.N; r.rid = n.rid; r.cid = n.cid; r.valid = 0;
         P[i] = r;
     }
     __syncwarp();
@@ -658,13 +688,10 @@
                                                          pslam_plane* __restrict__ abi_planes, int32_t* __restrict__ out_n,
                                                          int32_t* __restrict__ final_map, int32_t* __restrict__ status) {
     const int frame = blockIdx.x, tid = threadIdx.x;
-    __shared__ double s_st[PEAC_MAX_PLANES * 9];
-    __shared__ double s_geo[PEAC_MAX_PLANES * 8];
-    __shared__ int32_t s_n[PEAC_MAX_PLANES], s_rid[PEAC_MAX_PLANES], s_cid[PEAC_MAX_PLANES], s_nb[PEAC_MAX_PLANES];
+    __shared__ PeacNode s_node[PEAC_MAX_PLANES];
+    __shared__ PeacNodeCold s_cold[PEAC_MAX_PLANES];
     __shared__ uint16_t s_heap[PEAC_MAX_PLANES];
-    __shared__ uint8_t s_alive[PEAC_MAX_PLANES];
     __shared__ float s_key[PEAC_MAX_PLANES];
-    __shared__ int16_t s_wlo[PEAC_MAX_PLANES], s_whi[PEAC_MAX_PLANES];
     __shared__ uint16_t s_ex[PEAC_MAX_PLANES];
     PeacPlaneRec* P = planes + (size_t)frame * PEAC_MAX_PLANES;
     PeacPlaneRec* O = out_planes + (size_t)frame * PEAC_MAX_PLANES;
@@ -672,34 +699,36 @@
     const int np = n_planes[frame];
     const size_t fo = (size_t)frame * g.nblk;
     for (int i = tid; i < np; i += 32) {
-        for (int k = 0; k < 9; ++k) s_st[i * 9 + k] = P[i].st[k];
-        for (int k = 0; k < 3; ++k) { s_geo[i * 8 + k] = P[i].center[k]; s_geo[i * 8 + 3 + k] = P[i].normal[k]; }
-        s_geo[i * 8 + 6] = P[i].mse; s_geo[i * 8 + 7] = P[i].curvature;
-        s_n[i] = P[i].N; s_rid[i] = P[i].rid; s_cid[i] = P[i].cid; s_alive[i] = (uint8_t)P[i].valid;
-        s_key[i] = (float)P[i].mse; s_wlo[i] = 0; s_whi[i] = PEAC_PL_WORDS - 1;
+        PeacNode& n = s_node[i];
+        for (int k = 0; k < 9; ++k) n.st[k] = P[i].st[k];
+        for (int k = 0; k < 3; ++k) { s_cold[i].center[k] = P[i].center[k]; n.normal[k] = P[i].normal[k]; }
+        n.mse = P[i].mse; s_cold[i].curvature = P[i].curvature;
+        n.N = P[i].N; n.rid = P[i].rid; n.cid = P[i].cid; n.alive = P[i].valid;
+        s_key[i] = (float)P[i].mse; n.wlo = 0; n.whi = PEAC_PL_WORDS - 1;
     }
     for (int i = tid; i < PEAC_MAX_PLANES; i += 32) fmap[i] = -1;
     __syncwarp();
     AhcState S;
     S.nslots = np; S.words = PEAC_PL_WORDS;
-    S.st = s_st; S.geo = s_geo; S.N = s_n; S.rid = s_rid; S.cid = s_cid; S.alive = s_alive;
+    S.node = s_node; S.cold = s_cold;
     S.adj = pl_adj + (size_t)frame * PEAC_MAX_PLANES * PEAC_PL_WORDS;
-    S.heap = s_heap; S.keyf = s_key; S.wlo = s_wlo; S.whi = s_whi; S.nb_list = s_nb; S.ds_parent = ds_parent + fo; S.ds_size = ds_size + fo;
+    S.heap = s_heap; S.heap_key = s_key; S.ds_parent = ds_parent + fo; S.ds_size = ds_size + fo;
     int heap_len = 0;
-    if (tid == 0) { const HeapKey hkey{S.keyf, S.geo}; for (int i = 0; i < np; ++i) if (s_alive[i]) heap_push(S.heap, heap_len, hkey, i); }
+    if (tid == 0) heap_len = AhcHeap{S.heap, S.heap_key, S.node}.build(np, [&](int i) { return s_node[i].alive != 0; });
     heap_len = __shfl_sync(0xffffffffu, heap_len, 0);
     __syncwarp();
     int n_ex = 0, next_cid = next_cid_in[frame];
     bool overflow = false;
-    ahc_run(g, S, heap_len, next_cid, s_ex, 1, n_ex, overflow);
+    ahc_run<false>(g, S, heap_len, next_cid, s_ex, 1, n_ex, overflow);
     if (overflow && tid == 0) atomicOr(status + frame, 16);
     for (int j = tid; j < n_ex; j += 32) {
         const int s = s_ex[j];
         PeacPlaneRec r;
-        for (int k = 0; k < 3; ++k) { r.center[k] = s_geo[s * 8 + k]; r.normal[k] = s_geo[s * 8 + 3 + k]; }
-        r.mse = s_geo[s * 8 + 6]; r.curvature = s_geo[s * 8 + 7];
-        for (int k = 0; k < 9; ++k) r.st[k] = s_st[s * 9 + k];
-        r.N = s_n[s]; r.rid = s_rid[s]; r.cid = s_cid[s]; r.valid = 1;
+        const PeacNode& n = s_node[s];
+        for (int k = 0; k < 3; ++k) { r.center[k] = s_cold[s].center[k]; r.normal[k] = n.normal[k]; }
+        r.mse = n.mse; r.curvature = s_cold[s].curvature;
+        for (int k = 0; k < 9; ++k) r.st[k] = n.st[k];
+        r.N = n.N; r.rid = n.rid; r.cid = n.cid; r.valid = 1;
         O[j] = r;
         pslam_plane a;
         for (int k = 0; k < 3; ++k) { a.normal[k] = r.normal[k]; a.center[k] = r.center[k]; }
diff --git a/planarslam_b200/csrc/peac_pipeline.cu b/planarslam_b200/csrc/peac_pipeline.cu
--- a/planarslam_b200/csrc/peac_pipeline.cu
+++ b/planarslam_b200/csrc/peac_pipeline.cu
@@ -46,9 +46,7 @@
 #define A(call) if ((rc = (call)) != PSLAM_OK) return rc
     A(dmalloc(c, &c->d_depth, B * px));
     A(dmalloc(c, &c->d_blk_st, B * nb * 9)); A(dmalloc(c, &c->d_blk_geo, B * nb * 8)); A(dmalloc(c, &c->d_blk_n, B * nb)); A(dmalloc(c, &c->d_blk_valid, B * nb));
-    A(dmalloc(c, &c->d_node_st, B * nb * 9)); A(dmalloc(c, &c->d_node_geo, B * nb * 8)); A(dmalloc(c, &c->d_node_n, B * nb));
-    A(dmalloc(c, &c->d_node_rid, B * nb)); A(dmalloc(c, &c->d_node_cid, B * nb)); A(dmalloc(c, &c->d_node_alive, B * nb));
-    A(dmalloc(c, &c->d_adj, B * nb * g.adj_words)); A(dmalloc(c, &c->d_wlo, B * nb)); A(dmalloc(c, &c->d_whi, B * nb)); A(dmalloc(c, &c->d_nb_list, B * nb)); A(dmalloc(c, &c->d_keyf, B * nb));
+    A(dmalloc(c, &c->d_node, B * nb)); A(dmalloc(c, &c->d_node_cold, B * nb)); A(dmalloc(c, &c->d_adj, B * nb * g.adj_words));
     A(dmalloc(c, &c->d_ds_parent, B * nb)); A(dmalloc(c, &c->d_ds_size, B * nb));
     A(dmalloc(c, &c->d_coarse, B * PEAC_MAX_PLANES)); A(dmalloc(c, &c->d_ncoarse, B)); A(dmalloc(c, &c->d_next_cid, B)); A(dmalloc(c, &c->d_blk_map, B * nb));
     A(dmalloc(c, &c->d_dist, B * px)); A(dmalloc(c, &c->d_queue, B * g.queue_cap)); A(dmalloc(c, &c->d_qlen, B));
@@ -65,19 +63,14 @@
 
 void peac_free(pslam_ctx* c) {
     cudaFree(c->d_depth); cudaFree(c->d_blk_st); cudaFree(c->d_blk_geo); cudaFree(c->d_blk_n); cudaFree(c->d_blk_valid);
-    cudaFree(c->d_node_st); cudaFree(c->d_node_geo); cudaFree(c->d_node_n); cudaFree(c->d_node_rid); cudaFree(c->d_node_cid);
-    cudaFree(c->d_node_alive); cudaFree(c->d_adj); cudaFree(c->d_wlo); cudaFree(c->d_whi); cudaFree(c->d_nb_list); cudaFree(c->d_keyf); cudaFree(c->d_ds_parent); cudaFree(c->d_ds_size);
+    cudaFree(c->d_node); cudaFree(c->d_node_cold); cudaFree(c->d_adj); cudaFree(c->d_ds_parent); cudaFree(c->d_ds_size);
     cudaFree(c->d_coarse); cudaFree(c->d_ncoarse); cudaFree(c->d_next_cid); cudaFree(c->d_blk_map); cudaFree(c->d_dist); cudaFree(c->d_queue);
     cudaFree(c->d_qlen); cudaFree(c->d_pl_adj); cudaFree(c->d_final); cudaFree(c->d_scratch); cudaFree(c->d_final_map); cudaFree(c->d_labels); cudaFree(c->d_planes);
     cudaFree(c->d_nplanes); cudaFree(c->d_midx); cudaFree(c->d_moff); cudaFreeHost(c->h_depth);
 }
 
-static int peac_cluster_occ() {
-    static const int occ = [] { const char* e = std::getenv("PSLAM_PEAC_OCC"); const int v = e ? std::atoi(e) : 12; return (v == 16 || v == 20) ? v : 12; }();
-    return occ;
-}
-static size_t peac_cluster_smem(const PeacGeom& g, int occ) {
-    return (size_t)g.nblk * (occ > 12 ? sizeof(uint16_t) : sizeof(float) + sizeof(uint16_t));
+static size_t peac_cluster_smem(const PeacGeom& g) {
+    return (size_t)g.nblk * (sizeof(float) + sizeof(uint16_t));
 }
 
 int peac_run_dev(pslam_ctx* c, const uint16_t* d_depth, int nframes, int32_t* d_labels, pslam_plane* d_planes, int32_t* d_nplanes,
@@ -92,16 +85,11 @@
     PSLAM_CUDA(c, cudaMemsetAsync(c->d_adj, 0, (size_t)nframes * g.nblk * g.adj_words * sizeof(uint32_t), st));
     PSLAM_CUDA(c, cudaMemsetAsync(c->d_pl_adj, 0, (size_t)nframes * PEAC_MAX_PLANES * PEAC_PL_WORDS * sizeof(uint32_t), st));
     PSLAM_LAUNCH(c, "peac_blocks", k_peac_blocks<<<dim3((g.nblk + 127) / 128, nframes), 128, 0, st>>>(g, d_depth, c->d_blk_st, c->d_blk_geo, c->d_blk_n, c->d_blk_valid));
-    const int occ = peac_cluster_occ();
-    const size_t cluster_smem = peac_cluster_smem(g, occ);
-#define PEAC_CLUSTER(V) do { \
-        PSLAM_CUDA(c, cudaFuncSetAttribute(k_peac_cluster<V>, cudaFuncAttributeMaxDynamicSharedMemorySize, (int)cluster_smem)); \
-        PSLAM_CUDA(c, cudaFuncSetAttribute(k_peac_cluster<V>, cudaFuncAttributePreferredSharedMemoryCarveout, cudaSharedmemCarveoutMaxShared)); \
-        PSLAM_LAUNCH(c, "peac_cluster", k_peac_cluster<V><<<nframes, 32, cluster_smem, st>>>(g, c->d_blk_st, c->d_blk_geo, c->d_blk_n, c->d_blk_valid, c->d_node_st, \
-                     c->d_node_geo, c->d_node_n, c->d_node_rid, c->d_node_cid, c->d_node_alive, c->d_adj, c->d_wlo, c->d_whi, c->d_nb_list, c->d_ds_parent, c->d_ds_size, \
-                     c->d_coarse, c->d_ncoarse, c->d_blk_map, c->d_next_cid, c->d_status, c->d_keyf)); } while (0)
-    if (occ == 16) PEAC_CLUSTER(16); else if (occ == 20) PEAC_CLUSTER(20); else PEAC_CLUSTER(12);
-#undef PEAC_CLUSTER
+    const size_t cluster_smem = peac_cluster_smem(g);
+    PSLAM_CUDA(c, cudaFuncSetAttribute(k_peac_cluster, cudaFuncAttributeMaxDynamicSharedMemorySize, (int)cluster_smem));
+    PSLAM_CUDA(c, cudaFuncSetAttribute(k_peac_cluster, cudaFuncAttributePreferredSharedMemoryCarveout, cudaSharedmemCarveoutMaxShared));
+    PSLAM_LAUNCH(c, "peac_cluster", k_peac_cluster<<<nframes, 32, cluster_smem, st>>>(g, c->d_blk_st, c->d_blk_geo, c->d_blk_n, c->d_blk_valid, c->d_node,
+                 c->d_node_cold, c->d_adj, c->d_ds_parent, c->d_ds_size, c->d_coarse, c->d_ncoarse, c->d_blk_map, c->d_next_cid, c->d_status));
     PSLAM_LAUNCH(c, "peac_seed", k_peac_seed<<<nframes, 256, 0, st>>>(g, c->d_blk_map, d_labels, c->d_dist, c->d_queue, c->d_qlen));
     const size_t flood_smem = PEAC_MAX_PLANES * sizeof(FloodPlane) + (size_t)g.nblk;
     PSLAM_CUDA(c, cudaFuncSetAttribute(k_peac_flood, cudaFuncAttributeMaxDynamicSharedMemorySize, (int)flood_smem));
@@ -130,16 +118,12 @@
 
 int pslam_peac_wave_frames(const pslam_ctx* c) {
     if (!c) return 0;
-    const int occ = peac_cluster_occ();
-    const size_t cluster_smem = peac_cluster_smem(c->pgeom, occ);
+    const size_t cluster_smem = peac_cluster_smem(c->pgeom);
     int per_sm = 0, sms = 0, dev = 0;
     if (cudaGetDevice(&dev) != cudaSuccess) return 0;
-#define PEAC_OCCUPANCY(V) do { \
-        if (cudaFuncSetAttribute(k_peac_cluster<V>, cudaFuncAttributeMaxDynamicSharedMemorySize, (int)cluster_smem) != cudaSuccess) return 0; \
-        cudaFuncSetAttribute(k_peac_cluster<V>, cudaFuncAttributePreferredSharedMemoryCarveout, cudaSharedmemCarveoutMaxShared); \
-        if (cudaOccupancyMaxActiveBlocksPerMultiprocessor(&per_sm, k_peac_cluster<V>, 32, cluster_smem) != cudaSuccess) return 0; } while (0)
-    if (occ == 16) PEAC_OCCUPANCY(16); else if (occ == 20) PEAC_OCCUPANCY(20); else PEAC_OCCUPANCY(12);
-#undef PEAC_OCCUPANCY
+    if (cudaFuncSetAttribute(k_peac_cluster, cudaFuncAttributeMaxDynamicSharedMemorySize, (int)cluster_smem) != cudaSuccess) return 0;
+    cudaFuncSetAttribute(k_peac_cluster, cudaFuncAttributePreferredSharedMemoryCarveout, cudaSharedmemCarveoutMaxShared);
+    if (cudaOccupancyMaxActiveBlocksPerMultiprocessor(&per_sm, k_peac_cluster, 32, cluster_smem) != cudaSuccess) return 0;
     if (cudaDeviceGetAttribute(&sms, cudaDevAttrMultiProcessorCount, dev) != cudaSuccess) return 0;
     return per_sm * sms;
 }
diff --git a/planarslam_b200/csrc/pslam_internal.h b/planarslam_b200/csrc/pslam_internal.h
--- a/planarslam_b200/csrc/pslam_internal.h
+++ b/planarslam_b200/csrc/pslam_internal.h
@@ -71,6 +71,8 @@
 };
 
 struct PeacPlaneRec;
+struct PeacNode;
+struct PeacNodeCold;
 struct PoseBuffers;
 struct SearchBuffers;
 struct LbaBuffers;
@@ -123,9 +125,8 @@
     pslam::PeacGeom pgeom;
     uint16_t* d_depth = nullptr;
     double* d_blk_st = nullptr; double* d_blk_geo = nullptr; int32_t* d_blk_n = nullptr; uint8_t* d_blk_valid = nullptr;
-    double* d_node_st = nullptr; double* d_node_geo = nullptr; int32_t* d_node_n = nullptr; int32_t* d_node_rid = nullptr;
-    int32_t* d_node_cid = nullptr; uint8_t* d_node_alive = nullptr; uint32_t* d_adj = nullptr; int16_t* d_wlo = nullptr; int16_t* d_whi = nullptr;
-    int32_t* d_nb_list = nullptr; float* d_keyf = nullptr; int32_t* d_ds_parent = nullptr; int32_t* d_ds_size = nullptr;
+    pslam::PeacNode* d_node = nullptr; pslam::PeacNodeCold* d_node_cold = nullptr;
+    uint32_t* d_adj = nullptr; int32_t* d_ds_parent = nullptr; int32_t* d_ds_size = nullptr;
     pslam::PeacPlaneRec* d_coarse = nullptr; int32_t* d_ncoarse = nullptr; int32_t* d_next_cid = nullptr; int32_t* d_blk_map = nullptr;
     float* d_dist = nullptr; uint32_t* d_queue = nullptr; int32_t* d_qlen = nullptr; uint32_t* d_pl_adj = nullptr;
     pslam::PeacPlaneRec* d_final = nullptr; int32_t* d_scratch = nullptr; int32_t* d_final_map = nullptr;
```

After: 5267 (median of 6 runs). +1.8%, better.
